# liruiw/GA-DDPG

Hardware: AMD Instinct MI355X
Metric: DDPG grad-steps/sec (B=256, N=1024 pts) (higher is better)
Workload: dtype f32 (3xbf16-split products, f32 accumulate)

## Files before the change

ga-ddpg_amd/csrc/gemm.hip:

```cpp
#include "common.hpp"
#include <mutex>
#include <type_traits>
#include <string.h>

typedef float f32x16 __attribute__((ext_vector_type(16)));

#ifndef GAD_STREAM_STORE_AUX
#define GAD_STREAM_STORE_AUX 0
#endif

#define KT 32

__device__ __forceinline__ float4 f4zero() { return make_float4(0.f, 0.f, 0.f, 0.f); }
__device__ __forceinline__ float4 f4sel(bool c, float4 a, float4 b) {
    return make_float4(c ? a.x : b.x, c ? a.y : b.y, c ? a.z : b.z, c ? a.w : b.w);
}
__device__ __forceinline__ float4 ldg4(const float* p) { return *reinterpret_cast<const float4*>(p); }

typedef unsigned gad_u32x4 __attribute__((ext_vector_type(4)));
__device__ __forceinline__ float4 buf_ld4(__amdgpu_buffer_rsrc_t r, int vo, int so) {
    const gad_u32x4 u = __builtin_amdgcn_raw_buffer_load_b128(r, vo, so, 0);
    return make_float4(__uint_as_float(u.x), __uint_as_float(u.y), __uint_as_float(u.z), __uint_as_float(u.w));
}
__device__ __forceinline__ float buf_ld(__amdgpu_buffer_rsrc_t r, int vo, int so) {
// ... 511 lines not shown
    float4 rb[UB];
    auto load_tile = [&](int kt) {
        const int k0 = kt * KT;
        const bool tail = k0 + KT > bulk;
#pragma unroll
        for (int it = 0; it < UA; ++it) {
            int i, kk; unit_T<BM>(it * 256 + tid, i, kk);
            const int r = row0 + i;
            const bool ok = r < n_rows && (k0 + kk < Kp);
            ra[it] = x_raw<XM>(x, r, ok, zoff, k0 + kk, tail, XM == 1 ? ptS[i] : 0);
        }
#pragma unroll
        for (int it = 0; it < UB; ++it) {
            int j, kk; unit_T<BN>(it * 256 + tid, j, kk);
            const int n = n0 + j;
            const bool ok = n < n_out && (k0 + kk < Kp);
            rb[it] = ldg4(Wg + (size_t)(ok ? n : 0) * Kp + (ok ? k0 + kk : 0));
        }
    };
    auto store_tile = [&](int kt) {
        const int k0 = kt * KT;
#pragma unroll
        for (int it = 0; it < UA; ++it) {
            int i, kk; unit_T<BM>(it * 256 + tid, i, kk);
            const int r = row0 + i;
            const bool ok = r < n_rows && (k0 + kk < Kp);
            store_T<BM>(As, i, kk, x_finish<XM>(x, ra[it], ok, k0 + kk, sv, tv));
        }
#pragma unroll
        for (int it = 0; it < UB; ++it) {
            int j, kk; unit_T<BN>(it * 256 + tid, j, kk);
            const bool ok = (n0 + j) < n_out && (k0 + kk < Kp);
            store_T<BN>(Bs, j, kk, f4sel(ok, rb[it], f4zero()));
        }
    };
    bool preloaded = false;
    if (XM == 0) { load_tile(0); preloaded = true; }
    if (XM == 0 && x.affine) stage_affine<256>(sv, tv, x, zoff, x.c_in);
    for (; row0 < n_rows; row0 += gridDim.x * BM) {
        f32x16 acc[TM][TN];
#pragma unroll
        for (int a = 0; a < TM; ++a)
#pragma unroll
            for (int b = 0; b < TN; ++b)
#pragma unroll
                for (int v = 0; v < 16; ++v) acc[a][b][v] = 0.f;
        if (tid < BM) {
            const int r = row0 + tid;
            wS[tid] = r < n_rows ? (row_w ? row_w[r] : 1.f) : 0.f;
            if (XM == 1) ptS[tid] = r < n_rows ? x.row_pt[r] : 0;
        }
        int pgl = -1, pg_before = -1, pg_after = -1;
        float psgn = 1.f;
        if (POOL) {
            const int r = row0 + lane;
            pgl = r < n_rows ? pe.row_grp[r] : -1;
            pg_before = row0 > 0 ? pe.row_grp[row0 - 1] : -1;
            pg_after = row0 + BM < n_rows ? pe.row_grp[row0 + BM] : -1;
            psgn = pe.gamma[n0 + lane] < 0.f ? -1.f : 1.f;
        }
        __syncthreads();
        if (!preloaded) load_tile(0);
        preloaded = false;
        for (int kt = 0; kt < nk; ++kt) {
            store_tile(kt);
            __syncthreads();
            if (kt + 1 < nk) load_tile(kt + 1);
            mfma_ktile<TM, TN, PA, PB>(As, Bs, wm * TM * 32, wn * TN * 32, lane, acc);
            __syncthreads();
        }
        const int l31 = lane & 31, half = lane >> 5;
        if (POOL) {
            static_assert(!POOL || (BM == 64 && BN == 64 && TM == 1 && TN == 1 && TILE >= 64 * 65), "pooled epilogue: 64 x 64 tiles");
            float* zt = smem;
#pragma unroll
            for (int v = 0; v < 16; ++v) zt[(wm * 32 + acc_row(v, half)) * 65 + wn * 32 + l31] = acc[0][0][v];
            __syncthreads();
            {
                const float sg1[1] = {psgn};
                pool_tile64<1>(zt + lane, 65, 0, pgl, row0, min(64, n_rows - row0), sg1, __builtin_amdgcn_readfirstlane(wave), 4,
                               __builtin_amdgcn_readfirstlane(pg_before), __builtin_amdgcn_readfirstlane(pg_after),
                               pe.key + n0 + lane, pe.C);
            }
        }
#pragma unroll
        for (int tn = 0; tn < TN; ++tn) {
            const int n = n0 + wn * TN * 32 + tn * 32 + l31;
            float s1 = 0.f, s2 = 0.f;
#pragma unroll
            for (int tm = 0; tm < TM; ++tm)
#pragma unroll
                for (int v = 0; v < 16; ++v) {
                    const int il = wm * TM * 32 + tm * 32 + acc_row(v, half);
                    const int r = row0 + il;
                    const float zv = acc[tm][tn][v];
                    if (zout && r < n_rows && n < n_out) zout[(size_t)r * zout_pitch + ooff + n] = zv;
                    const float w = wS[il];
                    s1 = fmaf(w, zv, s1);
                    s2 = fmaf(w * zv, zv, s2);
                }
            csum[tn] += s1;
            csq[tn] += s2;
        }
        __syncthreads();
    }
    if (stat_sum) {
        const int rep = DET ? blockIdx.x : blockIdx.x % GAD_STAT_REPLICAS;
        block_column_atomics<WM, WN, TN, DET>(smem, csum, csq, lane, wm, wn, n0, n_out,
                                              stat_sum + (size_t)rep * stat_stride + ooff,
                                              stat_sq + (size_t)rep * stat_stride + ooff);
    }
}

typedef float f32x2 __attribute__((ext_vector_type(2)));

typedef __bf16 gad_bf16x8 __attribute__((ext_vector_type(8)));
__device__ __forceinline__ unsigned gad_cvt_pk_bf16(float lo, float hi) {
    unsigned r;
    __asm__("v_cvt_pk_bf16_f32 %0, %1, %2" : "=v"(r) : "v"(lo), "v"(hi));
    return r;
}
__device__ __forceinline__ void gad_split2(float a, float b, unsigned& H, unsigned& M, unsigned& L) {
    H = gad_cvt_pk_bf16(a, b);
    const f32x2 r = f32x2{a, b} - f32x2{__uint_as_float(H << 16), __uint_as_float(H & 0xffff0000u)};
    M = gad_cvt_pk_bf16(r.x, r.y);
    const f32x2 q = r - f32x2{__uint_as_float(M << 16), __uint_as_float(M & 0xffff0000u)};
    L = gad_cvt_pk_bf16(q.x, q.y);
}
__device__ __forceinline__ gad_bf16x8 gad_as_bf16x8(gad_u32x4 u) { return *reinterpret_cast<gad_bf16x8*>(&u); }

static int g_opt_mfma_split = 0;
static int g_opt_deterministic = 0;
static bool split_on(int family) {
    return !g_opt_deterministic && (g_opt_mfma_split == GAD_SPLIT_ALL || (g_opt_mfma_split & family) != 0);
}

namespace spw {
constexpr int APL = 64 * 64, BPL = 128 * 64, STAGE = 3 * (APL + BPL);
struct BRegs { gad_u32x4 r[2][3]; };
__device__ __forceinline__ void load_b(BRegs& b, __amdgpu_buffer_rsrc_t rs, const int (&vb)[2], int plane_bytes, int kt) {
#pragma unroll
    for (int u = 0; u < 2; ++u)
#pragma unroll
        for (int p = 0; p < 3; ++p) b.r[u][p] = __builtin_amdgcn_raw_buffer_load_b128(rs, vb[u], p * plane_bytes + kt * 64, 0);
}
__device__ __forceinline__ void store_b(unsigned char* stage, const BRegs& b, int tid) {
    const int row = tid >> 2;
    unsigned char* q = stage + 3 * APL + row * 64 + ((((tid & 3) ^ ((row >> 2) & 3))) << 4);
#pragma unroll
    for (int u = 0; u < 2; ++u)
#pragma unroll
        for (int p = 0; p < 3; ++p) *reinterpret_cast<gad_u32x4*>(q + p * BPL + u * (64 * 64)) = b.r[u][p];
}
__device__ __forceinline__ void store_a4(unsigned char* stage, int row, int tid, float4 v, unsigned sg) {
    unsigned h0, m0, l0, h1, m1, l1;
    gad_split2(__uint_as_float(__float_as_uint(v.x) ^ sg), __uint_as_float(__float_as_uint(v.y) ^ sg), h0, m0, l0);
    gad_split2(__uint_as_float(__float_as_uint(v.z) ^ sg), __uint_as_float(__float_as_uint(v.w) ^ sg), h1, m1, l1);
    unsigned char* q = stage + row * 64 + (((((tid & 7) >> 1) ^ ((row >> 2) & 3))) << 4) + ((tid & 1) << 3);
    *reinterpret_cast<uint2*>(q) = make_uint2(h0, h1);
    *reinterpret_cast<uint2*>(q + APL) = make_uint2(m0, m1);
    *reinterpret_cast<uint2*>(q + 2 * APL) = make_uint2(l0, l1);
}
__device__ __forceinline__ void ktile(const unsigned char* stage, int arow, int brow, int fo, f32x16 (&acc)[2], f32x16 (&an)[2]) {
#pragma unroll
    for (int s = 0; s < 2; ++s) {
        const int off = fo ^ (s << 5);
        const unsigned char* ap = stage + arow + off;
        const unsigned char* bp = stage + 3 * APL + brow + off;
        const gad_u32x4 AH = *reinterpret_cast<const gad_u32x4*>(ap), AM = *reinterpret_cast<const gad_u32x4*>(ap + APL);
        const gad_u32x4 AL = *reinterpret_cast<const gad_u32x4*>(ap + 2 * APL);
        gad_u32x4 BH[2], BM[2], BL[2];
#pragma unroll
        for (int t = 0; t < 2; ++t) {
            BH[t] = *reinterpret_cast<const gad_u32x4*>(bp + t * (32 * 64));
            BM[t] = *reinterpret_cast<const gad_u32x4*>(bp + BPL + t * (32 * 64));
            BL[t] = *reinterpret_cast<const gad_u32x4*>(bp + 2 * BPL + t * (32 * 64));
        }
#define GAD_SPW(A, B)                                                                                                          \
        _Pragma("unroll") for (int t = 0; t < 2; ++t) {                                                                        \
            if (s) an[t] = __builtin_amdgcn_mfma_f32_32x32x16_bf16(gad_as_bf16x8(A), gad_as_bf16x8(B[t]), an[t], 0, 0, 0);     \
            else acc[t] = __builtin_amdgcn_mfma_f32_32x32x16_bf16(gad_as_bf16x8(A), gad_as_bf16x8(B[t]), acc[t], 0, 0, 0);     \
        }
        GAD_SPW(AL, BH) GAD_SPW(AH, BL) GAD_SPW(AM, BM) GAD_SPW(AM, BH) GAD_SPW(AH, BM) GAD_SPW(AH, BH)
#undef GAD_SPW
    }
}
}

template <int XM, bool POOL, bool SP = false>
__global__ __launch_bounds__(256, 2) void gemm_fwd_wide_kernel(XSrc x, const int32_t* __restrict__ n_rows_dev, int n_rows_static,
                                                               const float* __restrict__ row_w, const float* __restrict__ W,
                                                               int Kp, int n_out, float* __restrict__ zout, int zout_pitch,
                                                               double* __restrict__ stat_sum, double* __restrict__ stat_sq,
                                                               int stat_stride, PoolEpi pe, const uint16_t* __restrict__ wsp,
                                                               int wsp_pitch, int wsp_plane, unsigned long long* __restrict__ ts) {
    KTimer kt_(ts);
    GAD_WPH_DECL;
    GAD_WKL_DECL;
    constexpr int BM = 64, BN = 128, P = KT + 4, STAGE = SP ? spw::STAGE / 4 : (BM + BN) * P, VM = 512;
    static_assert(2 * STAGE >= 64 * 129, "the pooled epilogue's tile lives in the operand buffers");
    __shared__ __attribute__((aligned(16))) float smem[2 * STAGE + 2 * VM + BM + 4 * BM];
    float* sv = smem + 2 * STAGE;
    float* tv = sv + VM;
    float* wS = tv + VM;
    float* dxS = wS + BM;
    const int tid = threadIdx.x, lane = tid & 63;
    const int wave = __builtin_amdgcn_readfirstlane(tid >> 6);
    const int wm = wave >> 1, wn = wave & 1;
    const int l31 = lane & 31, half = lane >> 5;
    const int n0 = blockIdx.y * BN;
    const int n_rows = n_rows_dev ? min(*n_rows_dev, n_rows_static) : n_rows_static;
    if ((int)(blockIdx.x * BM) >= n_rows) return;
    const int nk = (XM == 0 ? Kp : x.feat_c) / KT;
    const int c4 = (tid & 7) * 4;
    const int ur = tid >> 3;
    const __amdgpu_buffer_rsrc_t ar_ = __builtin_amdgcn_make_buffer_rsrc(const_cast<float*>(XM == 0 ? x.zin : x.feat), 0, GAD_BUF_MAX, 0x00020000);
    const __amdgpu_buffer_rsrc_t wr_ = __builtin_amdgcn_make_buffer_rsrc(const_cast<float*>(W), 0, GAD_BUF_MAX, 0x00020000);
    const int zo_pitch4 = zout_pitch * 4;
    const __amdgpu_buffer_rsrc_t zo_ = __builtin_amdgcn_make_buffer_rsrc(zout ? zout : const_cast<float*>(W), 0, zout ? gad_nbytes(n_rows, zo_pitch4) : 0, 0x00020000);
    int vb[4];
#pragma unroll
    for (int u = 0; u < 4; ++u) vb[u] = ((n0 + ur + 32 * u) * Kp + c4) * 4;
    const __amdgpu_buffer_rsrc_t ws_ = __builtin_amdgcn_make_buffer_rsrc(const_cast<uint16_t*>(SP ? wsp : reinterpret_cast<const uint16_t*>(W)), 0, GAD_BUF_MAX, 0x00020000);
    int vbs[2];
#pragma unroll
    for (int u = 0; u < 2; ++u) vbs[u] = ((n0 + (tid >> 2) + 64 * u) * wsp_pitch + (tid & 3) * 8) * 2;
    unsigned char* const smem_b = reinterpret_cast<unsigned char*>(smem);
    const int sp_fo = ((half ^ ((l31 >> 2) & 3)) << 4);
    if (XM == 0) {
        if (x.bn.stat_sum) {
            const bool writer = blockIdx.x == 0 && blockIdx.y == 0;
            for (int i = tid; i < Kp; i += 256) {
                float sc, sh;
                gad_bn_fin_channel(x.bn, i, writer, sc, sh);
                sv[i] = sc; tv[i] = sh;
            }
        } else {
            stage_affine<256>(sv, tv, x, 0, Kp);
        }
    }

    float csum[2] = {0.f, 0.f}, csq[2] = {0.f, 0.f};
    for (int row0 = blockIdx.x * BM; row0 < n_rows; row0 += gridDim.x * BM) {
        f32x16 acc[2];
        f32x16 an[2];
#pragma unroll
        for (int t = 0; t < 2; ++t)
#pragma unroll
            for (int v = 0; v < 16; ++v) { acc[t][v] = 0.f; if (SP) an[t][v] = 0.f; }
        int pgl = -1, pg_before = -1, pg_after = -1;
        float psgn[2] = {1.f, 1.f};
        if (POOL) {
            const int r = row0 + lane;
            pgl = r < n_rows ? pe.row_grp[r] : -1;
            pg_before = row0 > 0 ? pe.row_grp[row0 - 1] : -1;
            pg_after = row0 + BM < n_rows ? pe.row_grp[row0 + BM] : -1;
            psgn[0] = pe.gamma[n0 + lane] < 0.f ? -1.f : 1.f;
            psgn[1] = pe.gamma[n0 + 64 + lane] < 0.f ? -1.f : 1.f;
        }
        const int ra0 = min(row0 + ur, max(n_rows - 1, 0)), ra1 = min(row0 + ur + 32, max(n_rows - 1, 0));
        const int va0 = ((XM == 0 ? ra0 * x.zin_pitch : x.row_pt[ra0] * x.feat_c) + c4) * 4;
        const int va1 = ((XM == 0 ? ra1 * x.zin_pitch : x.row_pt[ra1] * x.feat_c) + c4) * 4;
        float4 ra2[2][2], rb2[2][SP ? 1 : 4];
        spw::BRegs rbs[SP ? 2 : 1];
        auto load_regs = [&](int kt, auto setc) {
            constexpr int S = decltype(setc)::value;
            const int k0 = kt * (KT * 4);
            ra2[S][0] = buf_ld4(ar_, va0, k0); ra2[S][1] = buf_ld4(ar_, va1, k0);
            if (SP) { spw::load_b(rbs[SP ? S : 0], ws_, vbs, wsp_plane * 2, kt); return; }
#pragma unroll
            for (int u = 0; u < (SP ? 1 : 4); ++u) rb2[S][u] = buf_ld4(wr_, vb[u], k0);
        };
        auto write_lds = [&](int kt, auto setc) {
            constexpr int S = decltype(setc)::value;
            const float4* ra = ra2[S];
            const float4* rb = rb2[S];
            float* As = smem + (kt & 1) * STAGE;
            float* Bs = As + BM * P;
            float4 s4 = make_float4(1.f, 1.f, 1.f, 1.f), t4 = f4zero();
            if (XM == 0) {
                s4 = *reinterpret_cast<const float4*>(sv + kt * KT + c4);
                t4 = *reinterpret_cast<const float4*>(tv + kt * KT + c4);
            }
#pragma unroll
            for (int u = 0; u < 2; ++u) {
                float4 v = ra[u];
                if (XM == 0) {
                    v.x = fmaxf(fmaf(v.x, s4.x, t4.x), 0.f); v.y = fmaxf(fmaf(v.y, s4.y, t4.y), 0.f);
                    v.z = fmaxf(fmaf(v.z, s4.z, t4.z), 0.f); v.w = fmaxf(fmaf(v.w, s4.w, t4.w), 0.f);
                }
                if (SP) spw::store_a4(smem_b + (kt & 1) * spw::STAGE, ur + 32 * u, tid, v, (ur & 1) ? 0x80000000u : 0u);
                else *reinterpret_cast<float4*>(As + (ur + 32 * u) * P + c4) = v;
            }
            if (SP) { spw::store_b(smem_b + (kt & 1) * spw::STAGE, rbs[SP ? S : 0], tid); return; }
#pragma unroll
            for (int u = 0; u < (SP ? 1 : 4); ++u) *reinterpret_cast<float4*>(Bs + (ur + 32 * u) * P + c4) = rb[u];
        };
        const std::integral_constant<int, 0> S0;
        const std::integral_constant<int, 1> S1;
        load_regs(0, S0);
        if (nk > 1) load_regs(1, S1);
        __syncthreads();
        if (tid < BM) {
            const int r = row0 + tid;
            wS[tid] = r < n_rows ? (row_w ? row_w[r] : 1.f) : 0.f;
            if (XM == 1) {
                const int rr = min(r, max(n_rows - 1, 0));
                const float* p = x.src_xyz + (size_t)x.row_pt[rr] * 3;
                float q0 = p[0], q1 = p[1], q2 = p[2];
                if (x.ctr_xyz) {
                    const float* cp = x.ctr_xyz + (size_t)x.row_grp[rr] * 3;
                    q0 = __fsub_rn(q0, cp[0]); q1 = __fsub_rn(q1, cp[1]); q2 = __fsub_rn(q2, cp[2]);
                }
                *reinterpret_cast<float4*>(dxS + 4 * tid) = make_float4(q0, q1, q2, 0.f);
            }
        }
        GAD_WPH(1);
        write_lds(0, S0);
        if (nk > 2) load_regs(2, S0);
        __syncthreads();
        GAD_WPH(2);
        auto ktile = [&](int kt, auto nxtc) {
            if (SP) {
                GAD_WKL(0);
                spw::ktile(smem_b + (kt & 1) * spw::STAGE, (wm * 32 + l31) * 64, (wn * 64 + l31) * 64, sp_fo, acc, an);
                GAD_WKL(1);
                if (kt + 1 < nk) write_lds(kt + 1, nxtc);
                if (kt + 3 < nk) load_regs(kt + 3, nxtc);
                GAD_WKL(2);
                __syncthreads();
                GAD_WKL(3);
                return;
            }
            const float* As = smem + (kt & 1) * STAGE + (wm * 32 + l31) * P + 4 * half;
            const float* Bs = smem + (kt & 1) * STAGE + BM * P + (wn * 64 + l31) * P + 4 * half;
            float4 a4 = *reinterpret_cast<const float4*>(As);
            float4 b0 = *reinterpret_cast<const float4*>(Bs), b1 = *reinterpret_cast<const float4*>(Bs + 32 * P);
#pragma unroll
            for (int j = 0; j < KT / 8; ++j) {
                float4 an = a4, bn0 = b0, bn1 = b1;
                if (j + 1 < KT / 8) {
                    an = *reinterpret_cast<const float4*>(As + 8 * (j + 1));
                    bn0 = *reinterpret_cast<const float4*>(Bs + 8 * (j + 1));
                    bn1 = *reinterpret_cast<const float4*>(Bs + 32 * P + 8 * (j + 1));
                }
                acc[0] = __builtin_amdgcn_mfma_f32_32x32x2f32(a4.x, b0.x, acc[0], 0, 0, 0);
                acc[1] = __builtin_amdgcn_mfma_f32_32x32x2f32(a4.x, b1.x, acc[1], 0, 0, 0);
                acc[0] = __builtin_amdgcn_mfma_f32_32x32x2f32(a4.y, b0.y, acc[0], 0, 0, 0);
                acc[1] = __builtin_amdgcn_mfma_f32_32x32x2f32(a4.y, b1.y, acc[1], 0, 0, 0);
                acc[0] = __builtin_amdgcn_mfma_f32_32x32x2f32(a4.z, b0.z, acc[0], 0, 0, 0);
                acc[1] = __builtin_amdgcn_mfma_f32_32x32x2f32(a4.z, b1.z, acc[1], 0, 0, 0);
                acc[0] = __builtin_amdgcn_mfma_f32_32x32x2f32(a4.w, b0.w, acc[0], 0, 0, 0);
                acc[1] = __builtin_amdgcn_mfma_f32_32x32x2f32(a4.w, b1.w, acc[1], 0, 0, 0);
                a4 = an; b0 = bn0; b1 = bn1;
            }
            if (kt + 1 < nk) write_lds(kt + 1, nxtc);
            if (kt + 3 < nk) load_regs(kt + 3, nxtc);
            __syncthreads();
        };
        for (int kt = 0; kt < nk; kt += 2) {
            ktile(kt, S1);
            if (kt + 1 < nk) ktile(kt + 1, S0);
        }
        GAD_WPH(3);
        if (SP) {
#pragma unroll
            for (int t = 0; t < 2; ++t)
#pragma unroll
                for (int v = 0; v < 16; ++v) acc[t][v] = (v & 1) ? an[t][v] - acc[t][v] : acc[t][v] - an[t][v];
        }
        if (XM == 1) {
#pragma unroll
            for (int t = 0; t < 2; ++t) {
                const float* wx = W + (size_t)(n0 + wn * 64 + t * 32 + l31) * Kp + x.feat_c;
                const float w0 = wx[0], w1 = wx[1], w2 = wx[2];
#pragma unroll
                for (int v = 0; v < 16; ++v) {
                    const float4 q = *reinterpret_cast<const float4*>(dxS + 4 * (wm * 32 + acc_row(v, half)));
                    acc[t][v] = fmaf(q.x, w0, fmaf(q.y, w1, fmaf(q.z, w2, acc[t][v])));
                }
            }
        }
        if (POOL) {
            float* zt = smem;
#pragma unroll
            for (int t = 0; t < 2; ++t)
#pragma unroll
                for (int v = 0; v < 16; ++v) zt[(wm * 32 + acc_row(v, half)) * 129 + wn * 64 + t * 32 + l31] = acc[t][v];
            __syncthreads();
            const int gb = __builtin_amdgcn_readfirstlane(pg_before), ga = __builtin_amdgcn_readfirstlane(pg_after);
            pool_tile64<2>(zt + lane, 129, 64, pgl, row0, min(64, n_rows - row0), psgn, wave, 4, gb, ga, pe.key + n0 + lane, pe.C);
        }
        if (SP) {
#pragma unroll
        for (int t = 0; t < 2; ++t) {
            const int n = n0 + wn * 64 + t * 32 + l31;
            const int vzo = (4 * half * zout_pitch + n) * 4;
#pragma unroll
            for (int v = 0; v < 16; ++v)
                __builtin_amdgcn_raw_buffer_store_b32(__float_as_uint(acc[t][v]), zo_, vzo, (row0 + wm * 32 + (v & 3) + 8 * (v >> 2)) * zo_pitch4, 0);
        }
        __builtin_amdgcn_sched_barrier(0);
#pragma unroll
        for (int t = 0; t < 2; ++t) {
            float s1 = 0.f, s2 = 0.f;
#pragma unroll
            for (int v = 0; v < 16; ++v) {
                const float w = wS[wm * 32 + acc_row(v, half)];
                const float zv = acc[t][v];
                s1 = fmaf(w, zv, s1);
                s2 = fmaf(w * zv, zv, s2);
            }
            csum[t] += s1;
            csq[t] += s2;
        }
        } else {
#pragma unroll
        for (int t = 0; t < 2; ++t) {
            const int n = n0 + wn * 64 + t * 32 + l31;
            const int vzo = (4 * half * zout_pitch + n) * 4;
            float s1 = 0.f, s2 = 0.f;
#pragma unroll
            for (int v = 0; v < 16; ++v) {
                const int il = wm * 32 + acc_row(v, half);
                const float zv = acc[t][v];
                __builtin_amdgcn_raw_buffer_store_b32(__float_as_uint(zv), zo_, vzo, (row0 + wm * 32 + (v & 3) + 8 * (v >> 2)) * zo_pitch4, 0);
                const float w = wS[il];
                s1 = fmaf(w, zv, s1);
                s2 = fmaf(w * zv, zv, s2);
            }
            csum[t] += s1;
            csq[t] += s2;
        }
        }
        GAD_WPH(4);
    }
    if (stat_sum) {
        const int rep = blockIdx.x % GAD_STAT_REPLICAS;
        block_column_atomics<2, 2, 2>(smem, csum, csq, lane, wm, wn, n0, n_out, stat_sum + (size_t)rep * stat_stride,
                                      stat_sq + (size_t)rep * stat_stride);
    }
#ifdef GAD_W_PHASES
    __asm__ volatile("s_waitcnt vmcnt(0)" ::: "memory");
    GAD_WPH(5);
    GAD_WPH_STORE(ts);
    GAD_WKL_STORE(ts);
#endif
}

static int g_opt_fwd_wide = 1;
static int g_opt_dx_wide = 1, g_opt_dw_wide = 1;
static int g_opt_bwd_fused = 1;
static int g_opt_fwd_bn_prologue = 1;
static int g_opt_bwd_wide = 0;
static int g_opt_bwd_wide_slab = 4;
static int g_opt_dw_wide_wgs = 256;
static bool fits_i32_bytes(long long rows, int pitch_a, int pitch_b, int pitch_c, int pitch_d);
static bool fwd_wideable(const gad_gemm_fwd_args& a) {
    if (g_opt_deterministic || !g_opt_fwd_wide || a.n_groups != 1 || a.zin_off[0] != 0 || a.w_off[0] != 0 || a.out_off[0] != 0) return false;
    if (!fits_i32_bytes(a.n_rows, a.mode == 1 ? a.feat_c : a.zin_pitch, a.zout ? a.zout_pitch : 0, 0, 0)) return false;
    if (a.n_rows < 2048 || a.n_out[0] % 128 != 0 || a.ones_col >= 0) return false;
    if (a.mode == 2) return false;
    if (a.mode == 1)
        return g_opt_fwd_wide != 2 && !a.pool_key && a.act_c == 0 && a.feat_c % 32 == 0 && a.feat_c >= 32 && a.feat_c <= 512 &&
               a.Kp == ((a.feat_c + 3 + 7) & ~7);
    if (a.Kp % 32 != 0 || a.Kp > 512 || a.Kp != a.c_in) return false;
    return !a.extra && a.scale && a.shift && a.relu;
}
static bool fits_i32_bytes(long long rows, int pitch_a, int pitch_b, int pitch_c, int pitch_d) {
    int p = pitch_a > pitch_b ? pitch_a : pitch_b;
    p = p > pitch_c ? p : pitch_c;
    p = p > pitch_d ? p : pitch_d;
    return rows * (long long)p * 4 <= (1ll << 31);
}

template <int KJ, int TN, int XM, bool POOL, bool SP = false>
__global__ __launch_bounds__(512, 2) void gemm_fwd_stream_kernel(XSrc x, const int32_t* __restrict__ n_rows_dev,
                                                                  int n_rows_static, const float* __restrict__ row_w,
// ... 16 lines not shown
    constexpr int PB = 2 * KP + 16;
    __shared__ __attribute__((aligned(16))) float Ws[SP ? 3 * NO * PB / 4 : NO * PW];
    __shared__ __attribute__((aligned(16))) float sv[KP], tv[KP];
    __shared__ float red[2 * 8 * NO];
    __shared__ float pz[POOL ? 8 * 32 * 64 : 1];
    static_assert(!POOL || TN == 4, "pooled epilogue: 128 output columns");
    const int tid = threadIdx.x, lane = tid & 63;
    const int wave = __builtin_amdgcn_readfirstlane(tid >> 6);
    const int l31 = lane & 31, half = lane >> 5;
    const int n_rows = n_rows_dev ? min(*n_rows_dev, n_rows_static) : n_rows_static;
    const int n_slabs = (n_rows + 31) >> 5;
#if GAD_X_PHASES == 2
    long long st1, st2, st3, st4;
    __asm__ volatile("s_waitcnt lgkmcnt(0)" ::: "memory");
    GAD_PH_STAMP(st1);
#endif
    int stride = gridDim.x * 8;
    int slab = wave * gridDim.x + blockIdx.x;
    int slab_end = n_slabs;
    if (POOL) {
        const int nw = gridDim.x * 8, base = n_slabs / nw, rem = n_slabs - base * nw;
        slab_end = slab * base + min(slab, rem) + base + (slab < rem ? 1 : 0);
        slab = slab * base + min(slab, rem);
        stride = 1;
    }
    const bool store_z = zout != nullptr;
    const __amdgpu_buffer_rsrc_t zrsrc =
        __builtin_amdgcn_make_buffer_rsrc(store_z ? zout : const_cast<float*>(W), 0, store_z ? gad_nbytes(n_rows, NO * 4) : 0, 0x00020000);
    const int zlane = (4 * half * NO + l31) * 4;
    float psgn[2];
    PoolRun prun[2];
    const int range0 = slab * 32;
    int g_after = -1;
    if (POOL && slab < slab_end) {
        const int g0 = pe.row_grp[range0];
        const int part0 = range0 > 0 && pe.row_grp[range0 - 1] == g0;
        if (slab_end * 32 < n_rows) g_after = pe.row_grp[slab_end * 32];
#pragma unroll
        for (int p = 0; p < 2; ++p) {
            psgn[p] = pe.gamma[p * 64 + lane] < 0.f ? -1.f : 1.f;
            prun[p].g = g0; prun[p].part = part0; prun[p].v = -INFINITY; prun[p].row = range0;
        }
    }

    f32x2 csum[TN], csq[TN];
#pragma unroll
    for (int t = 0; t < TN; ++t) { csum[t] = f32x2{0.f, 0.f}; csq[t] = f32x2{0.f, 0.f}; }

    XRaw ra[NG], rn[NG];
    float4 w1f[RE ? 2 : 1][RE ? PK : 1];
    if (RE) {
#pragma unroll
        for (int b = 0; b < 2; ++b)
#pragma unroll
            for (int j = 0; j < PK; ++j) w1f[b][j] = ldg4(x.pre_W + (size_t)(32 * b + l31) * x.pre_Kp + 8 * j + 4 * half);
    }
    int pt_nxt = 0;
    auto load_pt = [&](int sl) {
        const int r = min(sl * 32 + l31, max(n_rows - 1, 0));
        return (GATHER && sl < n_slabs) ? x.row_pt[r] : 0;
    };
    auto load_slab = [&](int sl, int pt, XRaw (&dst)[NG]) {
        const int r = min(sl < n_slabs ? sl * 32 + l31 : 0, max(n_rows - 1, 0));
        if (GATHER) {
            struct F3 { float x, y, z; } __attribute__((packed, aligned(4)));
            const float4 f = ldg4(x.feat + (size_t)pt * 4);
            const F3 p = *reinterpret_cast<const F3*>(x.src_xyz + (size_t)pt * 3);
            const int grp = x.row_grp[r];
            float q0 = p.x, q1 = p.y, q2 = p.z;
            if (x.ctr_xyz) {
                const F3 c = *reinterpret_cast<const F3*>(x.ctr_xyz + (size_t)grp * 3);
                q0 = __fsub_rn(q0, c.x); q1 = __fsub_rn(q1, c.y); q2 = __fsub_rn(q2, c.z);
            }
            float a0 = 0.f, a1 = 0.f, a2 = 0.f, a3 = 0.f, a4 = 0.f, a5 = 0.f;
            if (x.action) {
                const float* ap = x.action + (size_t)(grp / x.gps) * 6;
                const F3 u = *reinterpret_cast<const F3*>(ap), v = *reinterpret_cast<const F3*>(ap + 3);
                a0 = u.x; a1 = u.y; a2 = u.z; a3 = v.x; a4 = v.y; a5 = v.z;
            }
#pragma unroll
            for (int j = 0; j < NG; ++j) {
                dst[j].a = f;
                if (j == 0) dst[j].s = make_float4(q0, q1, q2, a0);
                else dst[j].s = half ? make_float4(a5, 0.f, 0.f, 0.f) : make_float4(a1, a2, a3, a4);
            }
            return;
        }
#pragma unroll
        for (int j = 0; j < NG; ++j)
            dst[j] = x_raw<GATHER ? 1 : 0>(x, r, true, 0, SP ? 16 * (j >> 1) + 8 * half + 4 * (j & 1) : 8 * j + 4 * half, GATHER, pt);
    };
    auto lds_b = [&](int j, float4 (&b4)[TN]) {
#pragma unroll
        for (int t = 0; t < TN; ++t) b4[t] = *reinterpret_cast<const float4*>(Ws + (t * 32 + l31) * PW + 8 * j + 4 * half);
    };
    {
        const int pt0 = load_pt(slab);
        load_slab(slab, pt0, ra);
        pt_nxt = load_pt(slab + stride);
    }
    {
        constexpr int UNITS = NO * KJ * 2, UW = (UNITS + 511) / 512;
        float4 wr[UW];
#pragma unroll
        for (int it = 0; it < UW; ++it) {
            const int u = it * 512 + tid;
            wr[it] = ldg4(W + (size_t)(u < UNITS ? u : 0) * 4);
        }
#if GAD_X_PHASES == 2
        GAD_PH_STAMP(st2);
        __asm__ volatile("s_waitcnt vmcnt(0)" ::: "memory");
        GAD_PH_STAMP(st3);
#endif
        if (ACT && tid < KP) {
            float sc, sh;
            if (x.bn.stat_sum) gad_bn_fin_channel(x.bn, tid, blockIdx.x == 0, sc, sh);
            else { sc = x.scale[tid]; sh = x.shift[tid]; }
            sv[tid] = sc; tv[tid] = sh;
        }
#pragma unroll
        for (int it = 0; it < UW; ++it) {
            const int u = it * 512 + tid;
            const int n = u / (KJ * 2), c = (u % (KJ * 2)) * 4;
            if (SP) {
                unsigned h0, m0, l0, h1, m1, l1;
                gad_split2(wr[it].x, wr[it].y, h0, m0, l0);
                gad_split2(wr[it].z, wr[it].w, h1, m1, l1);
                unsigned char* wp = reinterpret_cast<unsigned char*>(Ws) + n * PB + c * 2;
                if (u < UNITS) {
                    *reinterpret_cast<uint2*>(wp) = make_uint2(h0, h1);
                    *reinterpret_cast<uint2*>(wp + NO * PB) = make_uint2(m0, m1);
                    *reinterpret_cast<uint2*>(wp + 2 * NO * PB) = make_uint2(l0, l1);
                }
            } else if (u < UNITS) *reinterpret_cast<float4*>(Ws + n * PW + c) = wr[it];
        }
    }
    __syncthreads();
#if GAD_X_PHASES == 2
    GAD_PH_STAMP(st4);
    if (ts && lane == 0) {
        auto c16 = [&](long long t) { const long long d = (t - kt_start) >> 2; return (unsigned long long)(d > 65535 ? 65535 : d); };
        ts[2 * (blockIdx.x * 8 + wave)] = c16(st1) | (c16(st2) << 16) | (c16(st3) << 32) | (c16(st4) << 48);
    }
#endif

#ifdef GAD_X_PHASES
    long long tA = 0, tB = 0, tC = 0, ph_top = 0, ph_mfma = 0, ph_epi = 0;
    int ph_n = 0;
    long long tP, tS;
    GAD_PH_STAMP(tP);
    tS = (long long)kt_start;
#endif
    for (; slab < slab_end; slab += stride) {
        load_slab(slab + stride, pt_nxt, rn);
        pt_nxt = load_pt(slab + 2 * stride);
        float4 w4[4];
#pragma unroll
        for (int q = 0; q < 4; ++q) {
            const int r0 = slab * 32 + 8 * q + 4 * half;
            w4[q] = row_w ? ldg4(row_w + (r0 + 3 < n_rows_static ? r0 : 0)) : make_float4(1.f, 1.f, 1.f, 1.f);
        }
        if (slab * 32 + 32 > n_rows) {
#pragma unroll
            for (int q = 0; q < 4; ++q) {
                float* wq = &w4[q].x;
#pragma unroll
                for (int e = 0; e < 4; ++e) wq[e] = (slab * 32 + 8 * q + 4 * half + e < n_rows) ? wq[e] : 0.f;
            }
        }
        int gl = -1;
        if (POOL) { const int rr = slab * 32 + l31; gl = rr < n_rows ? pe.row_grp[rr] : -1; }
        __asm__ volatile("" ::: "memory");
        f32x16 acc[TN];
#pragma unroll
        for (int t = 0; t < TN; ++t)
#pragma unroll
            for (int v = 0; v < 16; ++v) acc[t][v] = 0.f;
        float4 bn[TN];
        if (!SP) lds_b(0, bn);
        GAD_PH_STAMP(tA);
        if (SP) {
            const unsigned char* wp = reinterpret_cast<const unsigned char*>(Ws) + l31 * PB + 16 * half;
            constexpr int NS = SP ? KJ / 2 : 1;
            gad_u32x4 AH[NS], AM[NS], AL[NS];
#pragma unroll
            for (int sg = 0; sg < NS; ++sg) {
                unsigned ah[4], am[4], al[4];
#pragma unroll
                for (int e = 0; e < 2; ++e) {
                    const int c = 16 * sg + 8 * half + 4 * e;
                    const float4 s4 = *reinterpret_cast<const float4*>(sv + c), t4 = *reinterpret_cast<const float4*>(tv + c);
                    const float4 zr = ra[SP ? 2 * sg + e : 0].a;
                    const float a0 = __builtin_fmaxf(fmaf(zr.x, s4.x, t4.x), 0.f), a1 = __builtin_fmaxf(fmaf(zr.y, s4.y, t4.y), 0.f);
                    const float a2 = __builtin_fmaxf(fmaf(zr.z, s4.z, t4.z), 0.f), a3 = __builtin_fmaxf(fmaf(zr.w, s4.w, t4.w), 0.f);
                    gad_split2(a0, a1, ah[2 * e], am[2 * e], al[2 * e]);
                    gad_split2(a2, a3, ah[2 * e + 1], am[2 * e + 1], al[2 * e + 1]);
                }
                const unsigned sgn = ((sg ^ l31) & 1) ? 0x80008000u : 0u;
                AH[sg] = gad_u32x4{ah[0] ^ sgn, ah[1] ^ sgn, ah[2] ^ sgn, ah[3] ^ sgn};
                AM[sg] = gad_u32x4{am[0] ^ sgn, am[1] ^ sgn, am[2] ^ sgn, am[3] ^ sgn};
                AL[sg] = gad_u32x4{al[0] ^ sgn, al[1] ^ sgn, al[2] ^ sgn, al[3] ^ sgn};
            }
#pragma unroll
            for (int pp = 0; pp < TN / 2; ++pp) {
                f32x16 an[2];
#pragma unroll
                for (int i = 0; i < 2; ++i)
#pragma unroll
                    for (int v = 0; v < 16; ++v) an[i][v] = 0.f;
#pragma unroll
                for (int sg = 0; sg < NS; ++sg) {
                    gad_u32x4 BH[2], BM[2], BL[2];
#pragma unroll
                    for (int i = 0; i < 2; ++i) {
                        const unsigned char* q = wp + (2 * pp + i) * 32 * PB + 32 * sg;
                        BH[i] = *reinterpret_cast<const gad_u32x4*>(q);
                        BM[i] = *reinterpret_cast<const gad_u32x4*>(q + NO * PB);
                        BL[i] = *reinterpret_cast<const gad_u32x4*>(q + 2 * NO * PB);
                    }
#define GAD_SPLIT_MFMA(A, B)                                                                                                   \
                    _Pragma("unroll") for (int i = 0; i < 2; ++i) {                                                             \
                        if (sg & 1) an[i] = __builtin_amdgcn_mfma_f32_32x32x16_bf16(gad_as_bf16x8(A[sg]), gad_as_bf16x8(B[i]), an[i], 0, 0, 0); \
                        else acc[2 * pp + i] = __builtin_amdgcn_mfma_f32_32x32x16_bf16(gad_as_bf16x8(A[sg]), gad_as_bf16x8(B[i]), acc[2 * pp + i], 0, 0, 0); \
                    }
                    GAD_SPLIT_MFMA(AL, BH) GAD_SPLIT_MFMA(AH, BL) GAD_SPLIT_MFMA(AM, BM)
                    GAD_SPLIT_MFMA(AM, BH) GAD_SPLIT_MFMA(AH, BM) GAD_SPLIT_MFMA(AH, BH)
#undef GAD_SPLIT_MFMA
                }
#pragma unroll
                for (int i = 0; i < 2; ++i)
#pragma unroll
                    for (int v = 0; v < 16; ++v) acc[2 * pp + i][v] = (v & 1) ? an[i][v] - acc[2 * pp + i][v] : acc[2 * pp + i][v] - an[i][v];
            }
        }
        f32x16 zacc[RE ? 2 : 1];
        if (RE) {
#pragma unroll
            for (int b = 0; b < 2; ++b)
#pragma unroll
                for (int v = 0; v < 16; ++v) zacc[b][v] = 0.f;
#pragma unroll
            for (int j = 0; j < PK; ++j) {
                const float4 xb = x_finish<1>(x, ra[j], true, 8 * j + 4 * half, sv, tv);
#pragma unroll
                for (int b = 0; b < 2; ++b) zacc[b] = __builtin_amdgcn_mfma_f32_32x32x2f32(w1f[b][j].x, xb.x, zacc[b], 0, 0, 0);
#pragma unroll
                for (int b = 0; b < 2; ++b) zacc[b] = __builtin_amdgcn_mfma_f32_32x32x2f32(w1f[b][j].y, xb.y, zacc[b], 0, 0, 0);
#pragma unroll
                for (int b = 0; b < 2; ++b) zacc[b] = __builtin_amdgcn_mfma_f32_32x32x2f32(w1f[b][j].z, xb.z, zacc[b], 0, 0, 0);
#pragma unroll
                for (int b = 0; b < 2; ++b) zacc[b] = __builtin_amdgcn_mfma_f32_32x32x2f32(w1f[b][j].w, xb.w, zacc[b], 0, 0, 0);
            }
        }
#pragma unroll
        for (int j = 0; j < (SP ? 0 : KJ); ++j) {
            float4 b4[TN];
#pragma unroll
            for (int t = 0; t < TN; ++t) b4[t] = bn[t];
            float4 a4;
            if (ACT) {
                const float4 s4 = *reinterpret_cast<const float4*>(sv + 8 * j + 4 * half);
                const float4 t4 = *reinterpret_cast<const float4*>(tv + 8 * j + 4 * half);
                float4 zr;
                if (RE) zr = make_float4(zacc[j >> 2][4 * (j & 3)], zacc[j >> 2][4 * (j & 3) + 1], zacc[j >> 2][4 * (j & 3) + 2],
                                         zacc[j >> 2][4 * (j & 3) + 3]);
                else zr = ra[RE ? 0 : j].a;
                const f32x2 lo = f32x2{zr.x, zr.y} * f32x2{s4.x, s4.y} + f32x2{t4.x, t4.y};
                const f32x2 hi = f32x2{zr.z, zr.w} * f32x2{s4.z, s4.w} + f32x2{t4.z, t4.w};
                a4 = make_float4(__builtin_fmaxf(lo.x, 0.f), __builtin_fmaxf(lo.y, 0.f), __builtin_fmaxf(hi.x, 0.f),
                                 __builtin_fmaxf(hi.y, 0.f));
            } else {
                a4 = x_finish<1>(x, ra[RE ? 0 : j], true, 8 * j + 4 * half, sv, tv);
            }
            if (j + 1 < KJ) lds_b(j + 1, bn);
#pragma unroll
            for (int t = 0; t < TN; ++t) acc[t] = __builtin_amdgcn_mfma_f32_32x32x2f32(a4.x, b4[t].x, acc[t], 0, 0, 0);
#pragma unroll
            for (int t = 0; t < TN; ++t) acc[t] = __builtin_amdgcn_mfma_f32_32x32x2f32(a4.y, b4[t].y, acc[t], 0, 0, 0);
#pragma unroll
            for (int t = 0; t < TN; ++t) acc[t] = __builtin_amdgcn_mfma_f32_32x32x2f32(a4.z, b4[t].z, acc[t], 0, 0, 0);
#pragma unroll
            for (int t = 0; t < TN; ++t) acc[t] = __builtin_amdgcn_mfma_f32_32x32x2f32(a4.w, b4[t].w, acc[t], 0, 0, 0);
        }
        GAD_PH_STAMP(tB);
        const int zrow = slab * 32 * NO * 4;
        if (POOL) {
            float* zt = pz + wave * (32 * 64);
#pragma unroll
            for (int p = 0; p < 2; ++p) {
#pragma unroll
                for (int v = 0; v < 16; ++v) {
                    zt[acc_row(v, half) * 64 + l31] = acc[2 * p][v];
                    zt[acc_row(v, half) * 64 + 32 + l31] = acc[2 * p + 1][v];
                }
                pool_scan32(zt + lane, 64, gl, slab * 32, psgn[p], prun[p], pe.key + p * 64 + lane, pe.C);
            }
        }
#pragma unroll
        for (int v = 0; v < 16; v += 2) {
            const int rb = ((v & 3) + 8 * (v >> 2)) * NO * 4;
            const f32x2 wr = f32x2{(&w4[v >> 2].x)[v & 3], (&w4[v >> 2].x)[(v & 3) + 1]};
#pragma unroll
            for (int t = 0; t < TN; ++t) {
                const f32x2 zv = f32x2{acc[t][v], acc[t][v + 1]};
                if (store_z) {
                    __builtin_amdgcn_raw_buffer_store_b32(__float_as_uint(acc[t][v]), zrsrc, zlane + t * 128, zrow + rb, GAD_STREAM_STORE_AUX);
                    __builtin_amdgcn_raw_buffer_store_b32(__float_as_uint(acc[t][v + 1]), zrsrc, zlane + t * 128, zrow + rb + NO * 4, GAD_STREAM_STORE_AUX);
                }
                const f32x2 wz = wr * zv;
                csum[t] += wz;
                csq[t] += wz * zv;
            }
        }
#pragma unroll
        for (int j = 0; j < NG; ++j) ra[j] = rn[j];
#ifdef GAD_X_PHASES
        GAD_PH_STAMP(tC);
        ph_top += tA - tP; ph_mfma += tB - tA; ph_epi += tC - tB; tP = tC; ++ph_n;
#endif
    }
#ifdef GAD_X_PHASES
    if (ts && lane == 0) {
        const unsigned w = blockIdx.x * 8 + wave;
        if (GAD_X_PHASES != 2) ts[2 * w] = ((unsigned long long)ph_mfma << 32) | (unsigned long long)(ph_epi & 0xffffffffu);
        ts[2 * w + 1] = ((unsigned long long)ph_top << 32) | ((unsigned long long)(tP - tS) & 0xffffff00u) | (unsigned long long)ph_n;
    }
#endif
    if (POOL && range0 < slab_end * 32) {
#pragma unroll
        for (int p = 0; p < 2; ++p)
            if (prun[p].g >= 0)
                pool_put(pe.key + p * 64 + lane, prun[p].g, pe.C, prun[p].v, prun[p].row, prun[p].part != 0 || prun[p].g == g_after);
    }
    if (stat_sum) {
#pragma unroll
        for (int t = 0; t < TN; ++t) {
            const float c0 = csum[t].x + csum[t].y, c1 = csq[t].x + csq[t].y;
            const float s0 = c0 + __shfl_xor(c0, 32, 64);
            const float s1 = c1 + __shfl_xor(c1, 32, 64);
            if (lane < 32) { red[wave * NO + t * 32 + lane] = s0; red[(8 + wave) * NO + t * 32 + lane] = s1; }
        }
        __syncthreads();
        if (tid < NO) {
            float s0 = 0.f, s1 = 0.f;
#pragma unroll
            for (int w = 0; w < 8; ++w) { s0 += red[w * NO + tid]; s1 += red[(8 + w) * NO + tid]; }
            const int rep = blockIdx.x % GAD_STAT_REPLICAS;
            atomic_add_f64(stat_sum + (size_t)rep * stat_stride + tid, (double)s0);
            atomic_add_f64(stat_sq + (size_t)rep * stat_stride + tid, (double)s1);
        }
    }
}

#define SK_NW 8
#define SK_CH 6
#define SK_SP 36
#define SK_KCAP (8 * SK_NW * SK_CH * SK_MAXCH)
#define SK_MAXCH 3
template <int NW>
__global__ __launch_bounds__(64 * NW) void gemm_fwd_skinny_kernel(XSrc x, Groups gr, int n_rows,
                                                                     const float* __restrict__ row_w,
                                                                     const float* __restrict__ W, int Kp,
                                                                     float* __restrict__ zout, int zout_pitch,
                                                                     double* __restrict__ stat_sum,
                                                                     double* __restrict__ stat_sq, int stat_stride, unsigned long long* __restrict__ ts) {
    KTimer kt(ts);
    __shared__ __attribute__((aligned(16))) float stA[NW * 32 * SK_SP], stW[NW * 32 * SK_SP];
    __shared__ __attribute__((aligned(16))) float sv[SK_KCAP], tv[SK_KCAP];
    float* const part = stA;
    static_assert(32 * SK_SP >= 16 * 64, "partial tile must fit the wavefront's stage");
    const int tid = threadIdx.x, lane = tid & 63;
    const int wave = __builtin_amdgcn_readfirstlane(tid >> 6);
    const int l31 = lane & 31, half = lane >> 5;
    const int g = blockIdx.z;
    const int zoff = gr.aoff[g], n_out = gr.nout[g], ooff = gr.ooff[g];
    const int n0 = blockIdx.x * 32, row0 = blockIdx.y * 32;
    if (n0 >= n_out) return;
    const float* Wg = W + gr.woff[g] + (size_t)min(n0 + l31, n_out - 1) * Kp + 4 * half;
    const int r = min(row0 + l31, max(n_rows - 1, 0));
    const int nj = Kp >> 3;
    const int per = (nj + NW - 1) / NW;
    const int j0 = wave * per, j1 = min(nj, j0 + per);

    f32x16 acc;
#pragma unroll
    for (int v = 0; v < 16; ++v) acc[v] = 0.f;
    float* const myA = stA + wave * (32 * SK_SP);
    float* const myW = stW + wave * (32 * SK_SP);
    const int rsub = lane >> 3, chunk = lane & 7;
    const float* pa[4];
    const float* pw[4];
#pragma unroll
    for (int i = 0; i < 4; ++i) {
        pa[i] = x.zin + (size_t)min(row0 + rsub + 8 * i, max(n_rows - 1, 0)) * x.zin_pitch + zoff + 4 * chunk;
        pw[i] = W + gr.woff[g] + (size_t)min(n0 + rsub + 8 * i, n_out - 1) * Kp + 4 * chunk;
    }
    auto staged = [&](int jb) { return jb + 4 <= j1 && 8 * (jb + 4) <= x.c_in; };
    float4 ga[4], gw[4];
    auto load_blk = [&](int jb) {
#pragma unroll
        for (int i = 0; i < 4; ++i) { ga[i] = ldg4(pa[i] + 8 * jb); gw[i] = ldg4(pw[i] + 8 * jb); }
    };
    if (j0 < j1 && staged(j0)) load_blk(j0);
    if (x.bn.stat_sum) {
        const bool writer = blockIdx.x == 0 && blockIdx.y == 0;
        for (int i = tid; i < x.c_in; i += 64 * NW) {
            float sc, sh;
            gad_bn_fin_channel(x.bn, i, writer, sc, sh);
            sv[i] = sc;
            tv[i] = sh;
        }
    } else if (x.affine) stage_affine<64 * NW>(sv, tv, x, zoff, x.c_in);
    __syncthreads();
    for (int jb = j0; jb < j1; jb += 4) {
        if (staged(jb)) {
#pragma unroll
            for (int i = 0; i < 4; ++i) {
                *reinterpret_cast<float4*>(myA + (rsub + 8 * i) * SK_SP + 4 * chunk) = ga[i];
                *reinterpret_cast<float4*>(myW + (rsub + 8 * i) * SK_SP + 4 * chunk) = gw[i];
            }
            if (jb + 4 < j1 && staged(jb + 4)) load_blk(jb + 4);
            __builtin_amdgcn_fence(__ATOMIC_RELEASE, "wavefront");
            __builtin_amdgcn_wave_barrier();
            __builtin_amdgcn_fence(__ATOMIC_ACQUIRE, "wavefront");
#pragma unroll
            for (int u = 0; u < 4; ++u) {
                XRaw raw;
                raw.a = *reinterpret_cast<const float4*>(myA + l31 * SK_SP + 8 * u + 4 * half);
                raw.s = f4zero();
                const float4 a4 = x_finish<0>(x, raw, true, 8 * (jb + u) + 4 * half, sv, tv);
                const float4 b4 = *reinterpret_cast<const float4*>(myW + l31 * SK_SP + 8 * u + 4 * half);
                acc = __builtin_amdgcn_mfma_f32_32x32x2f32(a4.x, b4.x, acc, 0, 0, 0);
                acc = __builtin_amdgcn_mfma_f32_32x32x2f32(a4.y, b4.y, acc, 0, 0, 0);
                acc = __builtin_amdgcn_mfma_f32_32x32x2f32(a4.z, b4.z, acc, 0, 0, 0);
                acc = __builtin_amdgcn_mfma_f32_32x32x2f32(a4.w, b4.w, acc, 0, 0, 0);
            }
            __builtin_amdgcn_fence(__ATOMIC_RELEASE, "wavefront");
            __builtin_amdgcn_wave_barrier();
        } else {
            const int je = min(jb + 4, j1);
            XRaw ra[4];
            float4 rb[4];
#pragma unroll
            for (int u = 0; u < 4; ++u) {
                const int j = min(jb + u, nj - 1);
                const int col = 8 * j + 4 * half;
                ra[u] = x_raw<0>(x, r, true, zoff, col, col + 4 > x.c_in, 0);
                rb[u] = ldg4(Wg + 8 * j);
            }
            if (jb + 4 < j1 && staged(jb + 4)) load_blk(jb + 4);
#pragma unroll
            for (int u = 0; u < 4; ++u) {
                if (jb + u < je) {
                    const float4 a4 = x_finish<0>(x, ra[u], true, 8 * (jb + u) + 4 * half, sv, tv);
                    const float4 b4 = rb[u];
                    acc = __builtin_amdgcn_mfma_f32_32x32x2f32(a4.x, b4.x, acc, 0, 0, 0);
                    acc = __builtin_amdgcn_mfma_f32_32x32x2f32(a4.y, b4.y, acc, 0, 0, 0);
                    acc = __builtin_amdgcn_mfma_f32_32x32x2f32(a4.z, b4.z, acc, 0, 0, 0);
                    acc = __builtin_amdgcn_mfma_f32_32x32x2f32(a4.w, b4.w, acc, 0, 0, 0);
                }
            }
        }
    }
#pragma unroll
    for (int v = 0; v < 16; ++v) part[wave * (32 * SK_SP) + v * 64 + lane] = acc[v];
    __syncthreads();
    if (wave != 0) return;
#pragma unroll
// ... 735 lines not shown
        };
        lds_operands(0);
        for (; quad < n_quads; quad += gridDim.x) {
            slab = quad * 4 + wave;
            const int r_nn = row_of(slab + 8 * gridDim.x);
            const int grp_nn = GM == 1 ? d.row_grp[r_nn] : 0;
            const float w_nxt = d.row_w ? d.row_w[r_nxt] : 1.f;
            const bool row_live = slab * 32 + l31 < n_rows;
            f32x16 acc[2];
#pragma unroll
            for (int t = 0; t < 2; ++t)
#pragma unroll
                for (int v = 0; v < 16; ++v) acc[t][v] = 0.f;
            float zp[2][16];
            const int zrow = (slab < n_slabs ? slab : 0) * 32 * 64 * 4;
#pragma unroll
            for (int uu = 0; uu < NU; ++uu) {
                if (uu + AHEAD < NU) load_u(r_cur, grp_cur, uu + AHEAD, (uu + AHEAD) % RING);
                else load_u(r_nxt, grp_nxt, uu + AHEAD - NU, (uu + AHEAD) % RING);
                if (uu == 0) {
#pragma unroll
                    for (int v = 0; v < 16; ++v)
#pragma unroll
                        for (int t = 0; t < 2; ++t)
                            zp[t][v] = __uint_as_float(__builtin_amdgcn_raw_buffer_load_b32(
                                zrsrc, glane + t * 128, zrow + ((v & 3) + 8 * (v >> 2)) * 256, 0));
                }
                __builtin_amdgcn_sched_barrier(0);
                float* const hb = mybuf + (uu / (NU / 2)) * (4 * 32 * HP) + (uu % (NU / 2)) * 8;
                {
                    const float4 z = rz[uu % RING];
                    float4 g = rg[uu % RING];
                    if (GM == 1) {
                        const int4 a = ra[uu % RING];
                        const int rr = slab * 32 + l31;
                        g.x = a.x == rr ? g.x : 0.f; g.y = a.y == rr ? g.y : 0.f;
                        g.z = a.z == rr ? g.z : 0.f; g.w = a.w == rr ? g.w : 0.f;
                    }
                    float4 a4;
                    a4.x = P.x * g.x - wrow * fmaf(S.x, z.x, Q.x); a4.y = P.y * g.y - wrow * fmaf(S.y, z.y, Q.y);
                    a4.z = P.z * g.z - wrow * fmaf(S.z, z.z, Q.z); a4.w = P.w * g.w - wrow * fmaf(S.w, z.w, Q.w);
                    if (!row_live) a4 = make_float4(0.f, 0.f, 0.f, 0.f);
                    *reinterpret_cast<float4*>(hb) = a4;
                    const float4 b0 = nb0, b1 = nb1;
                    lds_operands((uu + 1) % NU);
                    acc[0] = __builtin_amdgcn_mfma_f32_32x32x2f32(a4.x, b0.x, acc[0], 0, 0, 0);
                    acc[1] = __builtin_amdgcn_mfma_f32_32x32x2f32(a4.x, b1.x, acc[1], 0, 0, 0);
                    acc[0] = __builtin_amdgcn_mfma_f32_32x32x2f32(a4.y, b0.y, acc[0], 0, 0, 0);
                    acc[1] = __builtin_amdgcn_mfma_f32_32x32x2f32(a4.y, b1.y, acc[1], 0, 0, 0);
                    acc[0] = __builtin_amdgcn_mfma_f32_32x32x2f32(a4.z, b0.z, acc[0], 0, 0, 0);
                    acc[1] = __builtin_amdgcn_mfma_f32_32x32x2f32(a4.z, b1.z, acc[1], 0, 0, 0);
                    acc[0] = __builtin_amdgcn_mfma_f32_32x32x2f32(a4.w, b0.w, acc[0], 0, 0, 0);
                    acc[1] = __builtin_amdgcn_mfma_f32_32x32x2f32(a4.w, b1.w, acc[1], 0, 0, 0);
                }
                if ((uu + 1) % (NU / 2) == 0) __syncthreads();
            }
            const bool full = slab * 32 + 32 <= n_rows;
#pragma unroll
            for (int v = 0; v < 16; ++v) {
                const int row = acc_row(v, half);
                const bool live = slab * 32 + row < n_rows;
                const int rb = zrow + ((v & 3) + 8 * (v >> 2)) * 256;
#pragma unroll
                for (int t = 0; t < 2; ++t) {
                    const float gv = acc[t][v];
                    const float zv = zp[t][v];
                    const bool act = fmaf(zv, ps[t], pt[t]) > 0.f && live;
                    const float ga = act ? gv : 0.f;
                    if (full) __builtin_amdgcn_raw_buffer_store_b32(__float_as_uint(ga), grsrc, glane + t * 128, rb, GAD_STREAM_STORE_AUX);
                    else if (live) e.gout[(size_t)(slab * 32 + row) * 64 + t * 32 + l31] = ga;
                    sb[t] += ga;
                    sg[t] = fmaf(ga, (zv - pm[t]) * pi[t], sg[t]);
                }
            }
            r_cur = r_nxt; r_nxt = r_nn;
            grp_cur = grp_nxt; grp_nxt = grp_nn;
            wrow = w_nxt;
        }
#pragma unroll
        for (int t = 0; t < 2; ++t) {
            const float s0 = sb[t] + __shfl_xor(sb[t], 32, 64);
            const float s1 = sg[t] + __shfl_xor(sg[t], 32, 64);
            if (lane < 32) { red[wave * 64 + t * 32 + lane] = s0; red[(4 + wave) * 64 + t * 32 + lane] = s1; }
        }
    } else {
        const int q = wave - 4;
        const int b = q & 1;
        const int tcl = NCT == 2 ? (q >> 1) : 0;
        const int s0 = NCT == 2 ? 0 : 2 * (q >> 1);
        constexpr int NS = NCT == 2 ? 4 : 2;
        const float psb = e.ps[32 * b + l31], ptb = e.pt[32 * b + l31];
        f32x16 aw[2];
#pragma unroll
        for (int h = 0; h < 2; ++h)
#pragma unroll
            for (int v = 0; v < 16; ++v) aw[h][v] = 0.f;
        float yq[NS][16];
        auto load_y = [&](int slab, int s) {
            const int zrow = (slab < n_slabs ? slab : 0) * 32 * 64 * 4;
#pragma unroll
            for (int v = 0; v < 16; ++v)
                yq[s][v] = __uint_as_float(__builtin_amdgcn_raw_buffer_load_b32(zrsrc, glane + b * 128, zrow + ((v & 3) + 8 * (v >> 2)) * 256, 0));
        };
        const float* const rbase = dzb + (4 * half) * HP + 32 * tcl + l31;
#pragma unroll
        for (int s = 0; s < NS; ++s) load_y(blockIdx.x * 4 + s0 + s, s);
        for (int quad = blockIdx.x; quad < n_quads; quad += gridDim.x) {
#pragma unroll
            for (int h = 0; h < 2; ++h) {
                __syncthreads();
#pragma unroll
                for (int s = 0; s < NS; ++s) {
                    const float* rb = rbase + (h * 4 + s0 + s) * (32 * HP);
                    float dz[16];
#pragma unroll
                    for (int v = 0; v < 16; ++v) dz[v] = rb[((v & 3) + 8 * (v >> 2)) * HP];
                    if (h == 0) {
#pragma unroll
                        for (int v = 0; v < 16; ++v) yq[s][v] = fmaxf(fmaf(yq[s][v], psb, ptb), 0.f);
                    }
#pragma unroll
                    for (int v = 0; v < 16; ++v) aw[h] = __builtin_amdgcn_mfma_f32_32x32x2f32(dz[v], yq[s][v], aw[h], 0, 0, 0);
                    if (h == 1) load_y((quad + gridDim.x) * 4 + s0 + s, s);
                }
            }
        }
        float* pout = partial + (size_t)(NCT == 2 ? blockIdx.x : 2 * blockIdx.x + (q >> 1)) * NO * 64;
#pragma unroll
        for (int h = 0; h < 2; ++h)
#pragma unroll
            for (int v = 0; v < 16; ++v) pout[(32 * (NCT * h + tcl) + acc_row(v, half)) * 64 + 32 * b + l31] = aw[h][v];
    }
    __syncthreads();
    if (tid < 64) {
        float s0 = 0.f, s1 = 0.f;
#pragma unroll
        for (int w = 0; w < 4; ++w) { s0 += red[w * 64 + tid]; s1 += red[(4 + w) * 64 + tid]; }
        const int rep = blockIdx.x % GAD_STAT_REPLICAS;
        atomic_add_f64(e.dbeta + (size_t)rep * e.stat_stride + tid, (double)s0);
        atomic_add_f64(e.dgamma + (size_t)rep * e.stat_stride + tid, (double)s1);
    }
}

template <int NJ, int GM, bool DW>
__global__ __launch_bounds__(512, 2) void gemm_bwd_stream_split_kernel(DzSrc d, const int32_t* __restrict__ n_rows_dev, int n_rows_static,
                                                                        const uint16_t* __restrict__ wsp, int wsp_plane, DxEpi e,
                                                                        float* __restrict__ partial, unsigned long long* __restrict__ ts) {
    KTimer kt(ts);
    constexpr int NO = 8 * NJ, NS = NO / 16;
    constexpr int HC = NO / 2, NCT = HC / 32;
    constexpr int RB = 2 * NO + 16, WPL = 64 * RB;
    constexpr int XSL = HC * 64, XPL = 4 * XSL, XBUF = 3 * XPL;
    __shared__ __attribute__((aligned(16))) unsigned char WtS[3 * WPL];
    __shared__ __attribute__((aligned(16))) float vec[3 * NO];
    __shared__ float red[2 * 8 * 64];
    __shared__ __attribute__((aligned(16))) unsigned char dzb[DW ? 2 * XBUF : 16];
    const int tid = threadIdx.x, lane = tid & 63;
    const int wave = __builtin_amdgcn_readfirstlane(tid >> 6);
    const int l31 = lane & 31, half = lane >> 5;
    const int n_rows = n_rows_dev ? min(*n_rows_dev, n_rows_static) : n_rows_static;
    {
        constexpr int CPR = NO / 8, UNITS = 3 * 64 * CPR, UW = (UNITS + 511) / 512;
        gad_u32x4 wr[UW];
#pragma unroll
        for (int it = 0; it < UW; ++it) {
            const int u = it * 512 + tid, uc = u < UNITS ? u : 0;
            const int pl = uc / (64 * CPR), rem = uc % (64 * CPR);
            wr[it] = *reinterpret_cast<const gad_u32x4*>(wsp + (size_t)pl * wsp_plane + (size_t)rem * 8);
        }
#pragma unroll
        for (int it = 0; it < UW; ++it) {
            const int u = it * 512 + tid;
            const int pl = u / (64 * CPR), rem = u % (64 * CPR), k = rem / CPR, c = rem % CPR;
            if (u < UNITS) *reinterpret_cast<gad_u32x4*>(WtS + pl * WPL + k * RB + c * 16) = wr[it];
        }
    }
    for (int i = tid; i < NO; i += 512) {
        float P, Q, S;
        dz_coef(d, i, P, Q, S, first_workgroup());
        vec[i] = P; vec[NO + i] = Q; vec[2 * NO + i] = S;
    }
    __syncthreads();
    const int n_slabs = (n_rows + 31) >> 5;
    const int n_quads = (n_slabs + 3) >> 2;
    const __amdgpu_buffer_rsrc_t zrsrc =
        __builtin_amdgcn_make_buffer_rsrc(const_cast<float*>(e.zprev), 0, gad_nbytes(n_rows, 64 * 4), 0x00020000);
    const int glane = (4 * half * 64 + l31) * 4;
    const int nprod = DW ? 4 : 8;

    if (!DW || wave < 4) {
        float ps[2], pt[2], pm[2], pi[2];
#pragma unroll
        for (int tk = 0; tk < 2; ++tk) {
            const int k = tk * 32 + l31;
            ps[tk] = e.ps[k]; pt[tk] = e.pt[k]; pm[tk] = e.pm[k]; pi[tk] = e.pi[k];
        }
        const __amdgpu_buffer_rsrc_t grsrc = __builtin_amdgcn_make_buffer_rsrc(e.gout, 0, gad_nbytes(n_rows, 64 * 4), 0x00020000);
        float sb[2] = {0.f, 0.f}, sg[2] = {0.f, 0.f};
        constexpr int NU = NO / 8, RING = 8, AHEAD = 6, RINGG = GM == 1 ? 4 : RING, AHEADG = GM == 1 ? 2 : AHEAD;
        static_assert(NU % RING == 0 && NU % RINGG == 0, "a slab's entries must fill the rings a whole number of times");
        float4 rz[RING], rg[RINGG];
        int4 ra[RINGG];
        auto row_of = [&](int sl) { return min(sl < n_slabs ? sl * 32 + l31 : 0, max(n_rows - 1, 0)); };
        auto load_z = [&](int r, int uu) {
            const unsigned n = 16 * (uu >> 1) + 8 * half + 4 * (uu & 1);
            rz[uu % RING] = ldg4(d.z + ((unsigned)r * NO + n));
            if (GM == 0) rg[uu % RINGG] = ldg4(d.G + ((unsigned)r * NO + n));
        };
        auto load_g = [&](int grp, int uu) {
            const unsigned n = 16 * (uu >> 1) + 8 * half + 4 * (uu & 1);
            ra[uu % RINGG] = *reinterpret_cast<const int4*>(d.argmax + ((unsigned)grp * NO + n));
            rg[uu % RINGG] = ldg4(d.dout + ((unsigned)grp * NO + n));
        };
        const int round_stride = DW ? 4 * gridDim.x : 8 * gridDim.x;
        int slab = DW ? blockIdx.x * 4 + wave : wave * gridDim.x + blockIdx.x;
        const int slab_limit = DW ? n_quads * 4 : n_slabs;
        int r_cur = row_of(slab), r_nxt = row_of(slab + round_stride);
        int grp_cur = GM == 1 ? d.row_grp[r_cur] : 0, grp_nxt = GM == 1 ? d.row_grp[r_nxt] : 0;
        float wrow = d.row_w ? d.row_w[r_cur] : 1.f;
#pragma unroll
        for (int i = 0; i < AHEAD; ++i) load_z(r_cur, i);
        if (GM == 1) {
#pragma unroll
            for (int i = 0; i < AHEADG; ++i) load_g(grp_cur, i);
        }
        const unsigned psel = (l31 & 1) ? 0x03020706u : 0x05040100u;
        const unsigned rsg = (l31 & 1) ? 0x80000000u : 0u;
        const int xq = l31 >> 3, xin = ((l31 >> 1) & 3) * 4;
        const unsigned char* const wb = WtS + l31 * RB + 16 * half;
        for (; slab < slab_limit; slab += round_stride) {
            const int r_nn = row_of(slab + 2 * round_stride);
            const int grp_nn = GM == 1 ? d.row_grp[r_nn] : 0;
            const float w_nxt = d.row_w ? d.row_w[r_nxt] : 1.f;
            const bool row_live = slab * 32 + l31 < n_rows;
            f32x16 acc[2], an[2];
#pragma unroll
            for (int t = 0; t < 2; ++t)
#pragma unroll
                for (int v = 0; v < 16; ++v) { acc[t][v] = 0.f; an[t][v] = 0.f; }
            float zp[2][16];
            const int zrow = (slab < n_slabs ? slab : 0) * 32 * 64 * 4;
#pragma unroll
            for (int s2 = 0; s2 < NS; ++s2) {
#pragma unroll
                for (int ee = 0; ee < 2; ++ee) {
                    const int uu = 2 * s2 + ee + AHEAD;
                    if (uu < NU) load_z(r_cur, uu); else load_z(r_nxt, uu - NU);
                    if (GM == 1) {
                        const int ug = 2 * s2 + ee + AHEADG;
                        if (ug < NU) load_g(grp_cur, ug); else load_g(grp_nxt, ug - NU);
                    }
                }
                if (s2 == 0) {
#pragma unroll
                    for (int v = 0; v < 16; ++v)
#pragma unroll
                        for (int t = 0; t < 2; ++t)
                            zp[t][v] = __uint_as_float(__builtin_amdgcn_raw_buffer_load_b32(
                                zrsrc, glane + t * 128, zrow + ((v & 3) + 8 * (v >> 2)) * 256, 0));
                }
                __builtin_amdgcn_sched_barrier(0);
                gad_u32x4 BH[2], BM[2], BL[2];
#pragma unroll
                for (int t = 0; t < 2; ++t) {
                    const unsigned char* q = wb + t * (32 * RB) + 32 * s2;
                    BH[t] = *reinterpret_cast<const gad_u32x4*>(q);
                    BM[t] = *reinterpret_cast<const gad_u32x4*>(q + WPL);
                    BL[t] = *reinterpret_cast<const gad_u32x4*>(q + 2 * WPL);
                }
                unsigned ah[4], am[4], al[4];
#pragma unroll
                for (int ee = 0; ee < 2; ++ee) {
                    const int uu = 2 * s2 + ee;
                    const int n = 16 * s2 + 8 * half + 4 * ee;
                    const float4 P = *reinterpret_cast<const float4*>(vec + n);
                    const float4 Q = *reinterpret_cast<const float4*>(vec + NO + n);
                    const float4 S = *reinterpret_cast<const float4*>(vec + 2 * NO + n);
                    const float4 z = rz[uu % RING];
                    float4 g = rg[uu % RINGG];
                    if (GM == 1) {
                        const int4 a = ra[uu % RINGG];
                        const int rr = slab * 32 + l31;
                        g.x = a.x == rr ? g.x : 0.f; g.y = a.y == rr ? g.y : 0.f;
                        g.z = a.z == rr ? g.z : 0.f; g.w = a.w == rr ? g.w : 0.f;
                    }
                    float4 a4;
                    a4.x = P.x * g.x - wrow * fmaf(S.x, z.x, Q.x); a4.y = P.y * g.y - wrow * fmaf(S.y, z.y, Q.y);
                    a4.z = P.z * g.z - wrow * fmaf(S.z, z.z, Q.z); a4.w = P.w * g.w - wrow * fmaf(S.w, z.w, Q.w);
                    if (!row_live) a4 = make_float4(0.f, 0.f, 0.f, 0.f);
                    gad_split2(__uint_as_float(__float_as_uint(a4.x) ^ rsg), __uint_as_float(__float_as_uint(a4.y) ^ rsg), ah[2 * ee], am[2 * ee], al[2 * ee]);
                    gad_split2(__uint_as_float(__float_as_uint(a4.z) ^ rsg), __uint_as_float(__float_as_uint(a4.w) ^ rsg), ah[2 * ee + 1], am[2 * ee + 1], al[2 * ee + 1]);
                }
                const gad_u32x4 AH = {ah[0], ah[1], ah[2], ah[3]}, AM = {am[0], am[1], am[2], am[3]}, AL = {al[0], al[1], al[2], al[3]};
                if (DW) {
                    unsigned char* hb = dzb + (s2 / (NS / 2)) * XBUF + wave * XSL + xin;
                    const int cbase = (16 * s2 + 8 * half) % HC + (l31 & 1);
#pragma unroll
                    for (int i = 0; i < 4; ++i) {
                        const int cl = cbase + 2 * i;
                        unsigned char* q = hb + cl * 64 + ((xq ^ ((cl >> 2) & 3)) << 4);
                        const unsigned own[3] = {ah[i], am[i], al[i]};
#pragma unroll
                        for (int pl = 0; pl < 3; ++pl) {
                            const unsigned nbr = (unsigned)__builtin_amdgcn_update_dpp(0, (int)own[pl], 0xB1, 0xf, 0xf, false);
                            *reinterpret_cast<unsigned*>(q + pl * XPL) = __builtin_amdgcn_perm(nbr, own[pl], psel);
                        }
                    }
                }
#define GAD_SPB(A, B)                                                                                                          \
                _Pragma("unroll") for (int t = 0; t < 2; ++t) {                                                                \
                    if (s2 & 1) an[t] = __builtin_amdgcn_mfma_f32_32x32x16_bf16(gad_as_bf16x8(A), gad_as_bf16x8(B[t]), an[t], 0, 0, 0);   \
                    else acc[t] = __builtin_amdgcn_mfma_f32_32x32x16_bf16(gad_as_bf16x8(A), gad_as_bf16x8(B[t]), acc[t], 0, 0, 0); \
                }
                GAD_SPB(AL, BH) GAD_SPB(AH, BL) GAD_SPB(AM, BM) GAD_SPB(AM, BH) GAD_SPB(AH, BM) GAD_SPB(AH, BH)
#undef GAD_SPB
                if (DW && (s2 + 1) % (NS / 2) == 0) __syncthreads();
            }
            const bool full = slab * 32 + 32 <= n_rows;
#pragma unroll
            for (int v = 0; v < 16; ++v) {
                const int row = acc_row(v, half);
                const bool live = slab * 32 + row < n_rows;
                const int rb = zrow + ((v & 3) + 8 * (v >> 2)) * 256;
#pragma unroll
                for (int t = 0; t < 2; ++t) {
                    const float gv = (v & 1) ? an[t][v] - acc[t][v] : acc[t][v] - an[t][v];
                    const float zv = live ? zp[t][v] : 0.f;
                    const bool act = fmaf(zv, ps[t], pt[t]) > 0.f && live;
                    const float ga = act ? gv : 0.f;
                    if (full) __builtin_amdgcn_raw_buffer_store_b32(__float_as_uint(ga), grsrc, glane + t * 128, rb, GAD_STREAM_STORE_AUX);
                    else if (live) e.gout[(size_t)(slab * 32 + row) * 64 + t * 32 + l31] = ga;
                    sb[t] += ga;
                    sg[t] = fmaf(ga, (zv - pm[t]) * pi[t], sg[t]);
                }
            }
            r_cur = r_nxt; r_nxt = r_nn;
            grp_cur = grp_nxt; grp_nxt = grp_nn;
            wrow = w_nxt;
        }
#pragma unroll
        for (int t = 0; t < 2; ++t) {
            const float s0 = sb[t] + __shfl_xor(sb[t], 32, 64);
            const float s1 = sg[t] + __shfl_xor(sg[t], 32, 64);
            if (lane < 32) { red[wave * 64 + t * 32 + lane] = s0; red[(8 + wave) * 64 + t * 32 + lane] = s1; }
        }
    } else {
        const int q = wave - 4;
        const int b = q & 1;
        const int tcl = NCT == 2 ? (q >> 1) : 0;
        const int s0 = NCT == 2 ? 0 : 2 * (q >> 1);
        constexpr int NSC = NCT == 2 ? 4 : 2;
        const float psb = e.ps[32 * b + l31], ptb = e.pt[32 * b + l31];
        f32x16 aw[2], awn[2];
#pragma unroll
        for (int h = 0; h < 2; ++h)
#pragma unroll
            for (int v = 0; v < 16; ++v) { aw[h][v] = 0.f; awn[h][v] = 0.f; }
        const int ylane = (8 * half * 64 + 32 * b + l31) * 4;
        float yr[NSC][16];
        gad_u32x4 YH[NSC][2], YM[NSC][2], YL[NSC][2];
        auto load_y = [&](int slab, int sl) {
            const int zrow = (slab < n_slabs ? slab : 0) * 32 * 64 * 4;
#pragma unroll
            for (int v = 0; v < 16; ++v)
                yr[sl][v] = __uint_as_float(__builtin_amdgcn_raw_buffer_load_b32(zrsrc, ylane, zrow + (16 * (v >> 3) + (v & 7)) * 256, 0));
        };
        const int cl = 32 * tcl + l31;
        const unsigned char* const rbase = dzb + cl * 64;
        const int fo = ((half ^ ((cl >> 2) & 3)) << 4);
#pragma unroll
        for (int sl = 0; sl < NSC; ++sl) load_y(blockIdx.x * 4 + s0 + sl, sl);
        for (int quad = blockIdx.x; quad < n_quads; quad += gridDim.x) {
#pragma unroll
            for (int h = 0; h < 2; ++h) {
                __syncthreads();
#pragma unroll
                for (int sl = 0; sl < NSC; ++sl) {
                    if (h == 0) {
#pragma unroll
                        for (int st = 0; st < 2; ++st) {
                            unsigned yh[4], ym[4], yl[4];
#pragma unroll
                            for (int i = 0; i < 4; ++i) {
                                float y0 = fmaxf(fmaf(yr[sl][8 * st + 2 * i], psb, ptb), 0.f), y1 = fmaxf(fmaf(yr[sl][8 * st + 2 * i + 1], psb, ptb), 0.f);
                                if (st) y0 = -y0; else y1 = -y1;
                                gad_split2(y0, y1, yh[i], ym[i], yl[i]);
                            }
                            YH[sl][st] = gad_u32x4{yh[0], yh[1], yh[2], yh[3]};
                            YM[sl][st] = gad_u32x4{ym[0], ym[1], ym[2], ym[3]};
                            YL[sl][st] = gad_u32x4{yl[0], yl[1], yl[2], yl[3]};
                        }
                    }
                    const unsigned char* rb = rbase + h * XBUF + (s0 + sl) * XSL;
#pragma unroll
                    for (int st = 0; st < 2; ++st) {
                        const int off = fo ^ (st << 5);
                        const gad_u32x4 AH = *reinterpret_cast<const gad_u32x4*>(rb + off);
                        const gad_u32x4 AM = *reinterpret_cast<const gad_u32x4*>(rb + XPL + off);
                        const gad_u32x4 AL = *reinterpret_cast<const gad_u32x4*>(rb + 2 * XPL + off);
#define GAD_SPC(A, B)                                                                                                          \
                        if (st) awn[h] = __builtin_amdgcn_mfma_f32_32x32x16_bf16(gad_as_bf16x8(A), gad_as_bf16x8(B[sl][st]), awn[h], 0, 0, 0); \
                        else aw[h] = __builtin_amdgcn_mfma_f32_32x32x16_bf16(gad_as_bf16x8(A), gad_as_bf16x8(B[sl][st]), aw[h], 0, 0, 0);
                        GAD_SPC(AL, YH) GAD_SPC(AH, YL) GAD_SPC(AM, YM) GAD_SPC(AM, YH) GAD_SPC(AH, YM) GAD_SPC(AH, YH)
#undef GAD_SPC
                    }
                    if (h == 1) load_y((quad + gridDim.x) * 4 + s0 + sl, sl);
                }
            }
        }
        float* pout = partial + (size_t)(NCT == 2 ? blockIdx.x : 2 * blockIdx.x + (q >> 1)) * NO * 64;
#pragma unroll
        for (int h = 0; h < 2; ++h)
#pragma unroll
            for (int v = 0; v < 16; ++v) pout[(32 * (NCT * h + tcl) + acc_row(v, half)) * 64 + 32 * b + l31] = aw[h][v] - awn[h][v];
    }
    __syncthreads();
    if (tid < 64) {
        float s0 = 0.f, s1 = 0.f;
        for (int w = 0; w < nprod; ++w) { s0 += red[w * 64 + tid]; s1 += red[(8 + w) * 64 + tid]; }
        const int rep = blockIdx.x % GAD_STAT_REPLICAS;
        atomic_add_f64(e.dbeta + (size_t)rep * e.stat_stride + tid, (double)s0);
        atomic_add_f64(e.dgamma + (size_t)rep * e.stat_stride + tid, (double)s1);
    }
}

template <int GM, int SC, bool SP = false>
__global__ __launch_bounds__(256, 2) void gemm_dx_wide_kernel(DzSrc d, const int32_t* __restrict__ n_rows_dev, int n_rows_static,
                                                              const float* __restrict__ W, int Kp, int n_out, DxEpi e,
                                                              const uint16_t* __restrict__ wsp, int wsp_plane,
                                                              unsigned long long* __restrict__ ts) {
    KTimer kt_(ts);
    constexpr int BM = 64, BN = 128, P = KT + 4, PB = BN + 4, STAGE = SP ? spw::STAGE / 4 : BM * P + KT * PB, VM = 512;
    __shared__ __attribute__((aligned(16))) float smem[2 * STAGE + 3 * VM + BM];
    __shared__ int32_t ptS[BM];
    float* vP = smem + 2 * STAGE;
    float* wS = vP + 3 * VM;
    int32_t* grS = reinterpret_cast<int32_t*>(wS);
    const int tid = threadIdx.x, lane = tid & 63;
    const int wave = __builtin_amdgcn_readfirstlane(tid >> 6);
    const int wm = wave >> 1, wn = wave & 1;
    const int l31 = lane & 31, half = lane >> 5;
    const int k0out = blockIdx.y * BN;
    const int n_rows = n_rows_dev ? min(*n_rows_dev, n_rows_static) : n_rows_static;
    if ((int)(blockIdx.x * BM) >= n_rows) return;
    const int nk = n_out / KT;
    const int gpitch = GM == 0 ? d.g_pitch : d.c;
    const __amdgpu_buffer_rsrc_t zr = __builtin_amdgcn_make_buffer_rsrc(const_cast<float*>(d.z), 0, GAD_BUF_MAX, 0x00020000);
    const __amdgpu_buffer_rsrc_t gr_ = __builtin_amdgcn_make_buffer_rsrc(const_cast<float*>(GM == 0 ? d.G : d.dout), 0, GAD_BUF_MAX, 0x00020000);
    const __amdgpu_buffer_rsrc_t ar = __builtin_amdgcn_make_buffer_rsrc(const_cast<int32_t*>(GM == 0 ? d.row_grp : d.argmax), 0, GAD_BUF_MAX, 0x00020000);
    const __amdgpu_buffer_rsrc_t wr = __builtin_amdgcn_make_buffer_rsrc(const_cast<float*>(W), 0, GAD_BUF_MAX, 0x00020000);
    const int zp_pitch4 = SC ? 0 : e.zprev_pitch * 4, go_pitch4 = SC ? 0 : e.gout_pitch * 4;
    const __amdgpu_buffer_rsrc_t pr = __builtin_amdgcn_make_buffer_rsrc(const_cast<float*>(SC ? W : e.zprev), 0, SC ? 0 : gad_nbytes(n_rows, zp_pitch4), 0x00020000);
    const __amdgpu_buffer_rsrc_t or_ = __builtin_amdgcn_make_buffer_rsrc(SC ? const_cast<float*>(W) : e.gout, 0, SC ? 0 : gad_nbytes(n_rows, go_pitch4), 0x00020000);
    const int c4 = (tid & 7) * 4, ur = tid >> 3;
    const int bk4 = (tid & 31) * 4, bn = tid >> 5;
    int vw[4];
#pragma unroll
    for (int u = 0; u < 4; ++u) vw[u] = ((bn + 8 * u) * Kp + k0out + bk4) * 4;
    const __amdgpu_buffer_rsrc_t ws_ = __builtin_amdgcn_make_buffer_rsrc(const_cast<uint16_t*>(SP ? wsp : reinterpret_cast<const uint16_t*>(W)), 0, GAD_BUF_MAX, 0x00020000);
    int vbs[2];
#pragma unroll
    for (int u = 0; u < 2; ++u) vbs[u] = ((k0out + (tid >> 2) + 64 * u) * n_out + (tid & 3) * 8) * 2;
    unsigned char* const smem_b = reinterpret_cast<unsigned char*>(smem);
    const int sp_fo = ((half ^ ((l31 >> 2) & 3)) << 4);
    for (int i = tid; i < n_out; i += 256) {
        float Pc, Qc, Sc;
        dz_coef(d, i, Pc, Qc, Sc, first_workgroup());
        vP[i] = Pc; vP[VM + i] = Qc; vP[2 * VM + i] = Sc;
    }
    (void)grS;
    float ps[2] = {0.f, 0.f}, pt[2] = {0.f, 0.f}, pm[2] = {0.f, 0.f}, pi[2] = {0.f, 0.f};
#pragma unroll
    for (int t = 0; t < 2; ++t) {
        const int k = k0out + wn * 64 + t * 32 + l31;
        if (!SC) { ps[t] = e.ps[k]; pt[t] = e.pt[k]; pm[t] = e.pm[k]; pi[t] = e.pi[k]; }
    }
    float cb[2] = {0.f, 0.f}, cg[2] = {0.f, 0.f};
    for (int row0 = blockIdx.x * BM; row0 < n_rows; row0 += gridDim.x * BM) {
        f32x16 acc[2];
        f32x16 an[2];
#pragma unroll
        for (int t = 0; t < 2; ++t)
#pragma unroll
            for (int v = 0; v < 16; ++v) { acc[t][v] = 0.f; if (SP) an[t][v] = 0.f; }
        int vz[2], vg[2];
        float wrow[2];
        bool live[2];
#pragma unroll
        for (int u = 0; u < 2; ++u) {
            const int r = row0 + ur + 32 * u;
            live[u] = r < n_rows;
            const int rr = live[u] ? r : max(n_rows - 1, 0);
            wrow[u] = d.row_w ? d.row_w[rr] : 1.f;
            vz[u] = (rr * d.z_pitch + c4) * 4;
            vg[u] = ((GM == 1 ? d.row_grp[rr] : rr) * gpitch + c4) * 4;
        }
        float4 rz[2], rg[2], rb[SP ? 1 : 4];
        gad_u32x4 ra[2];
        spw::BRegs rbs;
        auto load_regs = [&](int kt) {
#pragma unroll
            for (int u = 0; u < 2; ++u) {
                rz[u] = buf_ld4(zr, vz[u], kt * (KT * 4));
                rg[u] = buf_ld4(gr_, vg[u], kt * (KT * 4));
                if (GM == 1) ra[u] = __builtin_amdgcn_raw_buffer_load_b128(ar, vg[u], kt * (KT * 4), 0);
            }
            if (SP) { spw::load_b(rbs, ws_, vbs, wsp_plane * 2, kt); return; }
#pragma unroll
            for (int u = 0; u < (SP ? 1 : 4); ++u) rb[u] = buf_ld4(wr, vw[u], kt * (KT * 4) * Kp);
        };
        auto write_lds = [&](int kt) {
            float* As = smem + (kt & 1) * STAGE;
            float* Bs = As + BM * P;
            const int nb = kt * KT + c4;
            const float4 P4 = *reinterpret_cast<const float4*>(vP + nb), Q4 = *reinterpret_cast<const float4*>(vP + VM + nb);
            const float4 S4 = *reinterpret_cast<const float4*>(vP + 2 * VM + nb);
#pragma unroll
            for (int u = 0; u < 2; ++u) {
                float4 g = rg[u];
                const float4 z = rz[u];
                if (GM == 1) {
                    const unsigned r = row0 + ur + 32 * u;
                    g.x = ra[u].x == r ? g.x : 0.f; g.y = ra[u].y == r ? g.y : 0.f;
                    g.z = ra[u].z == r ? g.z : 0.f; g.w = ra[u].w == r ? g.w : 0.f;
                }
                const float w = wrow[u];
                float4 v;
                v.x = P4.x * g.x - w * fmaf(S4.x, z.x, Q4.x); v.y = P4.y * g.y - w * fmaf(S4.y, z.y, Q4.y);
                v.z = P4.z * g.z - w * fmaf(S4.z, z.z, Q4.z); v.w = P4.w * g.w - w * fmaf(S4.w, z.w, Q4.w);
                if (!live[u]) v = f4zero();
                if (SP) spw::store_a4(smem_b + (kt & 1) * spw::STAGE, ur + 32 * u, tid, v, (ur & 1) ? 0x80000000u : 0u);
                else *reinterpret_cast<float4*>(As + (ur + 32 * u) * P + c4) = v;
            }
            if (SP) { spw::store_b(smem_b + (kt & 1) * spw::STAGE, rbs, tid); return; }
#pragma unroll
            for (int u = 0; u < (SP ? 1 : 4); ++u)
                *reinterpret_cast<float4*>(Bs + (bn + 8 * u) * PB + bk4) = rb[u];
        };
        load_regs(0);
        __syncthreads();
        if (SC && tid < BM) ptS[tid] = e.row_pt[min(row0 + tid, max(n_rows - 1, 0))];
        write_lds(0);
        if (nk > 1) load_regs(1);
        __syncthreads();
        for (int kt = 0; kt < nk; ++kt) {
            if (SP) {
                spw::ktile(smem_b + (kt & 1) * spw::STAGE, (wm * 32 + l31) * 64, (wn * 64 + l31) * 64, sp_fo, acc, an);
                if (kt + 1 < nk) write_lds(kt + 1);
                if (kt + 2 < nk) load_regs(kt + 2);
                __syncthreads();
                continue;
            }
            const float* As = smem + (kt & 1) * STAGE + (wm * 32 + l31) * P + 4 * half;
            const float* Bs = smem + (kt & 1) * STAGE + BM * P + (4 * half) * PB + wn * 64 + l31;
            float4 a4 = *reinterpret_cast<const float4*>(As);
            float4 b0 = make_float4(Bs[0], Bs[PB], Bs[2 * PB], Bs[3 * PB]);
            float4 b1 = make_float4(Bs[32], Bs[PB + 32], Bs[2 * PB + 32], Bs[3 * PB + 32]);
#pragma unroll
            for (int j = 0; j < KT / 8; ++j) {
                float4 an = a4, bn0 = b0, bn1 = b1;
                if (j + 1 < KT / 8) {
                    an = *reinterpret_cast<const float4*>(As + 8 * (j + 1));
                    const float* bq = Bs + 8 * (j + 1) * PB;
                    bn0 = make_float4(bq[0], bq[PB], bq[2 * PB], bq[3 * PB]);
                    bn1 = make_float4(bq[32], bq[PB + 32], bq[2 * PB + 32], bq[3 * PB + 32]);
                }
                acc[0] = __builtin_amdgcn_mfma_f32_32x32x2f32(a4.x, b0.x, acc[0], 0, 0, 0);
                acc[1] = __builtin_amdgcn_mfma_f32_32x32x2f32(a4.x, b1.x, acc[1], 0, 0, 0);
                acc[0] = __builtin_amdgcn_mfma_f32_32x32x2f32(a4.y, b0.y, acc[0], 0, 0, 0);
                acc[1] = __builtin_amdgcn_mfma_f32_32x32x2f32(a4.y, b1.y, acc[1], 0, 0, 0);
                acc[0] = __builtin_amdgcn_mfma_f32_32x32x2f32(a4.z, b0.z, acc[0], 0, 0, 0);
                acc[1] = __builtin_amdgcn_mfma_f32_32x32x2f32(a4.z, b1.z, acc[1], 0, 0, 0);
                acc[0] = __builtin_amdgcn_mfma_f32_32x32x2f32(a4.w, b0.w, acc[0], 0, 0, 0);
                acc[1] = __builtin_amdgcn_mfma_f32_32x32x2f32(a4.w, b1.w, acc[1], 0, 0, 0);
                a4 = an; b0 = bn0; b1 = bn1;
            }
            if (kt + 1 < nk) write_lds(kt + 1);
            if (kt + 2 < nk) load_regs(kt + 2);
            __syncthreads();
        }
        if (SP) {
#pragma unroll
            for (int t = 0; t < 2; ++t)
#pragma unroll
                for (int v = 0; v < 16; ++v) acc[t][v] = (v & 1) ? an[t][v] - acc[t][v] : acc[t][v] - an[t][v];
        }
        if (SC) {
#pragma unroll
            for (int t = 0; t < 2; ++t) {
                const int k = k0out + wn * 64 + t * 32 + l31;
#pragma unroll
                for (int v = 0; v < 16; ++v) {
                    const int il = wm * 32 + acc_row(v, half);
                    if (row0 + il < n_rows) atomic_add_f32(e.dfeat + (size_t)ptS[il] * e.feat_c + k, acc[t][v]);
                }
            }
            continue;
        }
        const int rb0 = row0 + wm * 32;
#pragma unroll
        for (int t = 0; t < 2; ++t) {
            const int kcol = k0out + wn * 64 + t * 32 + l31;
            const int vzp = (4 * half * e.zprev_pitch + kcol) * 4, vgo = (4 * half * e.gout_pitch + kcol) * 4;
            float zp[16];
#pragma unroll
            for (int v = 0; v < 16; ++v) zp[v] = buf_ld(pr, vzp, (rb0 + (v & 3) + 8 * (v >> 2)) * zp_pitch4);
            const float npm = -pm[t] * pi[t];
            float sb = 0.f, sg = 0.f;
#pragma unroll
            for (int v = 0; v < 16; ++v) {
                const float ga = fmaf(zp[v], ps[t], pt[t]) > 0.f ? acc[t][v] : 0.f;
                __builtin_amdgcn_raw_buffer_store_b32(__float_as_uint(ga), or_, vgo, (rb0 + (v & 3) + 8 * (v >> 2)) * go_pitch4, 0);
                sb += ga;
                sg = fmaf(ga, fmaf(zp[v], pi[t], npm), sg);
            }
            cb[t] += sb; cg[t] += sg;
        }
    }
    if (SC) return;
    const int rep = blockIdx.x % GAD_STAT_REPLICAS;
    block_column_atomics<2, 2, 2>(smem, cb, cg, lane, wm, wn, k0out, e.k_valid, e.dbeta + (size_t)rep * e.stat_stride,
                                  e.dgamma + (size_t)rep * e.stat_stride);
}

__global__ __launch_bounds__(256) void dx_action_stream_kernel(DzSrc d, const int32_t* __restrict__ n_rows_dev, int n_rows_static,
                                                               const float* __restrict__ W, int Kp, int c0, DxEpi e,
                                                               unsigned long long* __restrict__ ts) {
    KTimer kt(ts);
    const int tid = threadIdx.x, lane = tid & 63;
    const int n_rows = n_rows_dev ? min(*n_rows_dev, n_rows_static) : n_rows_static;
    const int n_waves = gridDim.x * 4;
    const int gw = blockIdx.x * 4 + (tid >> 6);
    int chunk = (n_rows + n_waves - 1) / n_waves;
    chunk = (chunk + 3) & ~3;
    const int r0 = gw * chunk, r1 = min(n_rows, r0 + chunk);
    if (r0 >= r1) return;
    const int sub = lane >> 4, c4 = (lane & 15) * 4;
    float4 P, Q, S;
    dz_coef(d, c4 + 0, P.x, Q.x, S.x); dz_coef(d, c4 + 1, P.y, Q.y, S.y);
    dz_coef(d, c4 + 2, P.z, Q.z, S.z); dz_coef(d, c4 + 3, P.w, Q.w, S.w);
    float4 wa[6];
#pragma unroll
    for (int a = 0; a < 6; ++a)
        wa[a] = make_float4(W[(size_t)(c4 + 0) * Kp + c0 + a], W[(size_t)(c4 + 1) * Kp + c0 + a], W[(size_t)(c4 + 2) * Kp + c0 + a],
                            W[(size_t)(c4 + 3) * Kp + c0 + a]);
    double run[6] = {0.0, 0.0, 0.0, 0.0, 0.0, 0.0};
    int cur = -1;
    auto flush = [&]() {
        if (cur >= 0 && lane == 0)
#pragma unroll
            for (int a = 0; a < 6; ++a) atomic_add_f64(e.daction + (size_t)cur * 6 + a, run[a]);
#pragma unroll
        for (int a = 0; a < 6; ++a) run[a] = 0.0;
    };
    for (int rb = r0; rb < r1; rb += 4) {
        const int r = rb + sub;
        const bool live = r < r1;
        const int rr = live ? r : r1 - 1;
        const float4 z = ldg4(d.z + (size_t)rr * d.z_pitch + c4);
        const float4 g = ldg4(d.G + (size_t)rr * d.g_pitch + c4);
        const float w = d.row_w ? d.row_w[rr] : 1.f;
        const int smp = e.row_grp[rr] / e.gps;
        float4 dz;
        dz.x = P.x * g.x - w * fmaf(S.x, z.x, Q.x); dz.y = P.y * g.y - w * fmaf(S.y, z.y, Q.y);
        dz.z = P.z * g.z - w * fmaf(S.z, z.z, Q.z); dz.w = P.w * g.w - w * fmaf(S.w, z.w, Q.w);
        float p[6];
#pragma unroll
        for (int a = 0; a < 6; ++a) {
            p[a] = fmaf(dz.x, wa[a].x, fmaf(dz.y, wa[a].y, fmaf(dz.z, wa[a].z, dz.w * wa[a].w)));
            p[a] = live ? p[a] : 0.f;
#pragma unroll
            for (int m = 8; m >= 1; m >>= 1) p[a] += __shfl_xor(p[a], m, 16);
        }
        const int s0 = __builtin_amdgcn_readlane(smp, 0), s1 = __builtin_amdgcn_readlane(smp, 16);
        const int s2 = __builtin_amdgcn_readlane(smp, 32), s3 = __builtin_amdgcn_readlane(smp, 48);
        if (s0 == s1 && s1 == s2 && s2 == s3) {
            if (s0 != cur) { flush(); cur = s0; }
#pragma unroll
            for (int a = 0; a < 6; ++a) {
                float t = p[a] + __shfl_xor(p[a], 16, 64);
                t += __shfl_xor(t, 32, 64);
                run[a] += (double)t;
            }
        } else {
            flush();
            cur = -1;
            if ((lane & 15) == 0 && live)
#pragma unroll
                for (int a = 0; a < 6; ++a) atomic_add_f64(e.daction + (size_t)smp * 6 + a, (double)p[a]);
        }
    }
    flush();
}

static bool dx_action_streamable(const gad_gemm_dx_args& a, bool vec) {
    if (g_opt_deterministic || !g_opt_dx_stream || !vec || a.n_groups != 1 || a.dz_off[0] != 0 || a.w_off[0] != 0) return false;
    if (a.epilogue != 1 || a.dfeat || !a.daction || a.act_c != 6 || !a.row_grp || a.n_rows < 32768 || a.n_out[0] != 64) return false;
    const gad_dz_src& d = a.dz;
    return d.gmode == 0 && d.G && d.z && d.z_pitch % 4 == 0 && d.g_pitch % 4 == 0 && d.premasked && d.coefP && d.coefQ && d.coefS &&
           a.feat_c + 3 + a.act_c <= a.Kp;
// ... 967 lines not shown
    if (r_begin >= r_end) return;
    for (int i = tid; i < BT; i += 256) {
        float Pc, Qc, Sc;
        dz_coef(d, n0 + i, Pc, Qc, Sc, blockIdx.y == 0 && k0 == 0);
        vP[i] = Pc; vP[VM + i] = Qc; vP[2 * VM + i] = Sc;
        if (XM == 0) { sv[i] = x.scale[k0 + i]; tv[i] = x.shift[k0 + i]; }
    }
    const bool coords = XM == 1 && k0 == 0;
    float wx[4][3];
#pragma unroll
    for (int j = 0; j < 4; ++j) { wx[j][0] = 0.f; wx[j][1] = 0.f; wx[j][2] = 0.f; }
    f32x16 acc[2][2];
#pragma unroll
    for (int a = 0; a < 2; ++a)
#pragma unroll
        for (int b = 0; b < 2; ++b)
#pragma unroll
            for (int v = 0; v < 16; ++v) acc[a][b][v] = 0.f;
    const int c4 = (tid & 31) * 4, sr = tid >> 5;
    const int gpitch = GM == 0 ? d.g_pitch : d.c;
    float4 rz[4], rg[4], rx[4];
    int4 ra[4];
    float rw[4], rd[4][3];
    int pq[4], gq[4];
    int gd[4];
    auto load_idx = [&](int rb0) {
#pragma unroll
        for (int u = 0; u < 4; ++u) {
            const int r = rb0 + sr + 8 * u;
            const int rr = r < r_end ? r : r_end - 1;
            pq[u] = XM == 1 ? x.row_pt[rr] : 0;
            gq[u] = (XM == 1 && x.ctr_xyz) ? x.row_grp[rr] : 0;
            gd[u] = GM == 1 ? d.row_grp[rr] : 0;
        }
    };
    auto load_regs = [&](int rb0) {
#pragma unroll
        for (int u = 0; u < 4; ++u) {
            const int r = rb0 + sr + 8 * u;
            const int rr = r < r_end ? r : r_end - 1;
            rw[u] = d.row_w ? d.row_w[rr] : 1.f;
            rz[u] = ldg4(d.z + (size_t)rr * d.z_pitch + n0 + c4);
            if (GM == 0) {
                rg[u] = ldg4(d.G + (size_t)rr * gpitch + n0 + c4);
            } else {
                const int grp = gd[u];
                ra[u] = *reinterpret_cast<const int4*>(d.argmax + (size_t)grp * gpitch + n0 + c4);
                rg[u] = ldg4(d.dout + (size_t)grp * gpitch + n0 + c4);
            }
            if (XM == 0) {
                rx[u] = ldg4(x.zin + (size_t)rr * x.zin_pitch + k0 + c4);
            } else {
                rx[u] = ldg4(x.feat + (size_t)pq[u] * x.feat_c + k0 + c4);
                if (coords) {
                    const float* p = x.src_xyz + (size_t)pq[u] * 3;
                    float q0 = p[0], q1 = p[1], q2 = p[2];
                    if (x.ctr_xyz) {
                        const float* cp = x.ctr_xyz + (size_t)gq[u] * 3;
                        q0 = __fsub_rn(q0, cp[0]); q1 = __fsub_rn(q1, cp[1]); q2 = __fsub_rn(q2, cp[2]);
                    }
                    rd[u][0] = q0; rd[u][1] = q1; rd[u][2] = q2;
                }
            }
        }
        if (XM == 1 || GM == 1) load_idx(rb0 + KT);
    };
    auto write_lds = [&](int it, int rb0) {
        float* As = smem + (it & 1) * STAGE;
        float* Bs = As + KT * P;
        const float4 Pv = *reinterpret_cast<const float4*>(vP + c4), Qv = *reinterpret_cast<const float4*>(vP + VM + c4);
        const float4 Sv = *reinterpret_cast<const float4*>(vP + 2 * VM + c4);
        float4 s4 = f4zero(), t4 = f4zero();
        if (XM == 0) { s4 = *reinterpret_cast<const float4*>(sv + c4); t4 = *reinterpret_cast<const float4*>(tv + c4); }
#pragma unroll
        for (int u = 0; u < 4; ++u) {
            const int r = rb0 + sr + 8 * u;
            float4 g = rg[u];
            const float4 z = rz[u];
            if (GM == 1) {
                g.x = ra[u].x == r ? g.x : 0.f; g.y = ra[u].y == r ? g.y : 0.f;
                g.z = ra[u].z == r ? g.z : 0.f; g.w = ra[u].w == r ? g.w : 0.f;
            }
            const float w = rw[u];
            float4 a, b;
            a.x = Pv.x * g.x - w * fmaf(Sv.x, z.x, Qv.x); a.y = Pv.y * g.y - w * fmaf(Sv.y, z.y, Qv.y);
            a.z = Pv.z * g.z - w * fmaf(Sv.z, z.z, Qv.z); a.w = Pv.w * g.w - w * fmaf(Sv.w, z.w, Qv.w);
            if (XM == 0) {
                b.x = fmaxf(fmaf(rx[u].x, s4.x, t4.x), 0.f); b.y = fmaxf(fmaf(rx[u].y, s4.y, t4.y), 0.f);
                b.z = fmaxf(fmaf(rx[u].z, s4.z, t4.z), 0.f); b.w = fmaxf(fmaf(rx[u].w, s4.w, t4.w), 0.f);
            } else {
                b = rx[u];
            }
            if (r >= r_end) { a = f4zero(); b = f4zero(); }
            if (coords) {
#pragma unroll
                for (int dd = 0; dd < 3; ++dd) {
                    wx[0][dd] = fmaf(a.x, rd[u][dd], wx[0][dd]); wx[1][dd] = fmaf(a.y, rd[u][dd], wx[1][dd]);
                    wx[2][dd] = fmaf(a.z, rd[u][dd], wx[2][dd]); wx[3][dd] = fmaf(a.w, rd[u][dd], wx[3][dd]);
                }
            }
            *reinterpret_cast<float4*>(As + (sr + 8 * u) * P + c4) = a;
            *reinterpret_cast<float4*>(Bs + (sr + 8 * u) * P + c4) = b;
        }
    };
    if (XM == 1 || GM == 1) load_idx(r_begin);
    load_regs(r_begin);
    __syncthreads();
    write_lds(0, r_begin);
    if (r_begin + KT < r_end) load_regs(r_begin + KT);
    __syncthreads();
    int it = 0;
    for (int rb0 = r_begin; rb0 < r_end; rb0 += KT, ++it) {
        const float* As = smem + (it & 1) * STAGE + half * P + wm * 64 + l31;
        const float* Bs = smem + (it & 1) * STAGE + KT * P + half * P + wn * 64 + l31;
#pragma unroll
        for (int s = 0; s < KT / 2; ++s) {
            const float a0 = As[2 * s * P], a1 = As[2 * s * P + 32];
            const float b0 = Bs[2 * s * P], b1 = Bs[2 * s * P + 32];
            acc[0][0] = __builtin_amdgcn_mfma_f32_32x32x2f32(a0, b0, acc[0][0], 0, 0, 0);
            acc[0][1] = __builtin_amdgcn_mfma_f32_32x32x2f32(a0, b1, acc[0][1], 0, 0, 0);
            acc[1][0] = __builtin_amdgcn_mfma_f32_32x32x2f32(a1, b0, acc[1][0], 0, 0, 0);
            acc[1][1] = __builtin_amdgcn_mfma_f32_32x32x2f32(a1, b1, acc[1][1], 0, 0, 0);
        }
        if (rb0 + KT < r_end) write_lds(it + 1, rb0 + KT);
        if (rb0 + 2 * KT < r_end) load_regs(rb0 + 2 * KT);
        __syncthreads();
    }
    float* pout = partial + (size_t)blockIdx.y * n_out * Kp;
#pragma unroll
    for (int a = 0; a < 2; ++a)
#pragma unroll
        for (int b = 0; b < 2; ++b)
#pragma unroll
            for (int v = 0; v < 16; ++v) {
                const int n = n0 + wm * 64 + a * 32 + acc_row(v, half), k = k0 + wn * 64 + b * 32 + l31;
                pout[(size_t)n * Kp + k] = acc[a][b][v];
            }
    if (coords) {
        float* red = smem;
#pragma unroll
        for (int j = 0; j < 4; ++j)
#pragma unroll
            for (int dd = 0; dd < 3; ++dd) red[(sr * BT + c4 + j) * 3 + dd] = wx[j][dd];
        __syncthreads();
        for (int i = tid; i < BT * 3; i += 256) {
            float sum = 0.f;
#pragma unroll
            for (int q = 0; q < 8; ++q) sum += red[q * BT * 3 + i];
            pout[(size_t)(n0 + i / 3) * Kp + x.feat_c + i % 3] = sum;
        }
    }
}

template <int XM, int GM>
__global__ __launch_bounds__(256, 1) void gemm_dw_wide_split_kernel(DzSrc d, XSrc x, const int32_t* __restrict__ n_rows_dev,
                                                                    int n_rows_static, int Kp, int n_out, int tiles_k,
                                                                    float* __restrict__ partial, unsigned long long* __restrict__ ts) {
    KTimer kt_(ts);
    constexpr int BT = 128, OPL = BT * 64, STAGE = 6 * OPL, VM = 512;
    __shared__ __attribute__((aligned(16))) unsigned char smem_b[2 * STAGE];
    __shared__ __attribute__((aligned(16))) float vP[5 * VM];
    float* sv = vP + 3 * VM;
    float* tv = sv + VM;
    const int tid = threadIdx.x, lane = tid & 63;
    const int wave = __builtin_amdgcn_readfirstlane(tid >> 6);
    const int wm = wave >> 1, wn = wave & 1;
    const int l31 = lane & 31, half = lane >> 5;
    const int n0 = (blockIdx.x / tiles_k) * BT, k0 = (blockIdx.x % tiles_k) * BT;
    const int n_rows = n_rows_dev ? min(*n_rows_dev, n_rows_static) : n_rows_static;
    int chunk = gad_cdiv_dev(n_rows, (int)gridDim.y);
    chunk = (chunk + KT - 1) / KT * KT;
    const int r_begin = blockIdx.y * chunk, r_end = min(r_begin + chunk, n_rows);
    if (r_begin >= r_end) return;
    for (int i = tid; i < BT; i += 256) {
        float Pc, Qc, Sc;
        dz_coef(d, n0 + i, Pc, Qc, Sc, blockIdx.y == 0 && k0 == 0);
        vP[i] = Pc; vP[VM + i] = Qc; vP[2 * VM + i] = Sc;
        if (XM == 0) { sv[i] = x.scale[k0 + i]; tv[i] = x.shift[k0 + i]; }
    }
    const bool coords = XM == 1 && k0 == 0;
    float wx[4][3];
#pragma unroll
    for (int j = 0; j < 4; ++j) { wx[j][0] = 0.f; wx[j][1] = 0.f; wx[j][2] = 0.f; }
    f32x16 acc[2][2], an[2][2];
#pragma unroll
    for (int a = 0; a < 2; ++a)
#pragma unroll
        for (int b = 0; b < 2; ++b)
#pragma unroll
            for (int v = 0; v < 16; ++v) { acc[a][b][v] = 0.f; an[a][b][v] = 0.f; }
    const int rq = tid & 7, c4 = (tid >> 3) * 4;
    const float sgn = rq >= 4 ? -1.f : 1.f;
    const int gpitch = GM == 0 ? d.g_pitch : d.c;
    float4 rz[4], rg[4], rx[4];
    int4 ra[4];
    float rw[4], rd[4][3];
    int pq[4], gq[4], gd[4];
    auto load_idx = [&](int rb0) {
#pragma unroll
        for (int u = 0; u < 4; ++u) {
            const int r = rb0 + 4 * rq + u;
            const int rr = r < r_end ? r : r_end - 1;
            pq[u] = XM == 1 ? x.row_pt[rr] : 0;
            gq[u] = (XM == 1 && x.ctr_xyz) ? x.row_grp[rr] : 0;
            gd[u] = GM == 1 ? d.row_grp[rr] : 0;
        }
    };
    auto load_regs = [&](int rb0) {
#pragma unroll
        for (int u = 0; u < 4; ++u) {
            const int r = rb0 + 4 * rq + u;
            const int rr = r < r_end ? r : r_end - 1;
            rw[u] = d.row_w ? d.row_w[rr] : 1.f;
            rz[u] = ldg4(d.z + (size_t)rr * d.z_pitch + n0 + c4);
            if (GM == 0) {
                rg[u] = ldg4(d.G + (size_t)rr * gpitch + n0 + c4);
            } else {
                const int grp = gd[u];
                ra[u] = *reinterpret_cast<const int4*>(d.argmax + (size_t)grp * gpitch + n0 + c4);
                rg[u] = ldg4(d.dout + (size_t)grp * gpitch + n0 + c4);
            }
            if (XM == 0) {
                rx[u] = ldg4(x.zin + (size_t)rr * x.zin_pitch + k0 + c4);
            } else {
                rx[u] = ldg4(x.feat + (size_t)pq[u] * x.feat_c + k0 + c4);
                if (coords) {
                    const float* p = x.src_xyz + (size_t)pq[u] * 3;
                    float q0 = p[0], q1 = p[1], q2 = p[2];
                    if (x.ctr_xyz) {
                        const float* cp = x.ctr_xyz + (size_t)gq[u] * 3;
                        q0 = __fsub_rn(q0, cp[0]); q1 = __fsub_rn(q1, cp[1]); q2 = __fsub_rn(q2, cp[2]);
                    }
                    rd[u][0] = q0; rd[u][1] = q1; rd[u][2] = q2;
                }
            }
        }
        if (XM == 1 || GM == 1) load_idx(rb0 + KT);
    };
    const int wr_off = c4 * 64 + (rq & 1) * 8, wr_q = rq >> 1;
    auto write_lds = [&](int it, int rb0) {
        unsigned char* As = smem_b + (it & 1) * STAGE;
        unsigned char* Bs = As + 3 * OPL;
        const float4 Pv = *reinterpret_cast<const float4*>(vP + c4), Qv = *reinterpret_cast<const float4*>(vP + VM + c4);
        const float4 Sv = *reinterpret_cast<const float4*>(vP + 2 * VM + c4);
        float4 s4 = f4zero(), t4 = f4zero();
        if (XM == 0) { s4 = *reinterpret_cast<const float4*>(sv + c4); t4 = *reinterpret_cast<const float4*>(tv + c4); }
        float av[4][4], bv[4][4];
#pragma unroll
        for (int u = 0; u < 4; ++u) {
            const int r = rb0 + 4 * rq + u;
            float4 g = rg[u];
            const float4 z = rz[u];
            if (GM == 1) {
                g.x = ra[u].x == r ? g.x : 0.f; g.y = ra[u].y == r ? g.y : 0.f;
                g.z = ra[u].z == r ? g.z : 0.f; g.w = ra[u].w == r ? g.w : 0.f;
            }
            const float w = rw[u];
            float4 a, b;
            a.x = Pv.x * g.x - w * fmaf(Sv.x, z.x, Qv.x); a.y = Pv.y * g.y - w * fmaf(Sv.y, z.y, Qv.y);
            a.z = Pv.z * g.z - w * fmaf(Sv.z, z.z, Qv.z); a.w = Pv.w * g.w - w * fmaf(Sv.w, z.w, Qv.w);
            if (XM == 0) {
                b.x = fmaxf(fmaf(rx[u].x, s4.x, t4.x), 0.f); b.y = fmaxf(fmaf(rx[u].y, s4.y, t4.y), 0.f);
                b.z = fmaxf(fmaf(rx[u].z, s4.z, t4.z), 0.f); b.w = fmaxf(fmaf(rx[u].w, s4.w, t4.w), 0.f);
            } else {
                b = rx[u];
            }
            if (r >= r_end) { a = f4zero(); b = f4zero(); }
            if (coords) {
#pragma unroll
                for (int dd = 0; dd < 3; ++dd) {
                    wx[0][dd] = fmaf(a.x, rd[u][dd], wx[0][dd]); wx[1][dd] = fmaf(a.y, rd[u][dd], wx[1][dd]);
                    wx[2][dd] = fmaf(a.z, rd[u][dd], wx[2][dd]); wx[3][dd] = fmaf(a.w, rd[u][dd], wx[3][dd]);
                }
            }
            av[u][0] = a.x * sgn; av[u][1] = a.y * sgn; av[u][2] = a.z * sgn; av[u][3] = a.w * sgn;
            bv[u][0] = b.x; bv[u][1] = b.y; bv[u][2] = b.z; bv[u][3] = b.w;
        }
#pragma unroll
        for (int j = 0; j < 4; ++j) {
            const int off = wr_off + j * 64 + (((wr_q ^ (((c4 + j) >> 2) & 3))) << 4);
            unsigned h0, m0, l0, h1, m1, l1;
            gad_split2(av[0][j], av[1][j], h0, m0, l0);
            gad_split2(av[2][j], av[3][j], h1, m1, l1);
            *reinterpret_cast<uint2*>(As + off) = make_uint2(h0, h1);
            *reinterpret_cast<uint2*>(As + OPL + off) = make_uint2(m0, m1);
            *reinterpret_cast<uint2*>(As + 2 * OPL + off) = make_uint2(l0, l1);
            gad_split2(bv[0][j], bv[1][j], h0, m0, l0);
            gad_split2(bv[2][j], bv[3][j], h1, m1, l1);
            *reinterpret_cast<uint2*>(Bs + off) = make_uint2(h0, h1);
            *reinterpret_cast<uint2*>(Bs + OPL + off) = make_uint2(m0, m1);
            *reinterpret_cast<uint2*>(Bs + 2 * OPL + off) = make_uint2(l0, l1);
        }
    };
    if (XM == 1 || GM == 1) load_idx(r_begin);
    load_regs(r_begin);
    __syncthreads();
    write_lds(0, r_begin);
    if (r_begin + KT < r_end) load_regs(r_begin + KT);
    __syncthreads();
    const int fo = ((half ^ ((l31 >> 2) & 3)) << 4);
    const int arow = (wm * 64 + l31) * 64, brow = 3 * OPL + (wn * 64 + l31) * 64;
    int it = 0;
    for (int rb0 = r_begin; rb0 < r_end; rb0 += KT, ++it) {
        const unsigned char* st = smem_b + (it & 1) * STAGE;
#pragma unroll
        for (int s2 = 0; s2 < 2; ++s2) {
            const int off = fo ^ (s2 << 5);
            gad_u32x4 A[2][3], B[2][3];
#pragma unroll
            for (int a = 0; a < 2; ++a)
#pragma unroll
                for (int pl = 0; pl < 3; ++pl) {
                    A[a][pl] = *reinterpret_cast<const gad_u32x4*>(st + arow + a * (32 * 64) + pl * OPL + off);
                    B[a][pl] = *reinterpret_cast<const gad_u32x4*>(st + brow + a * (32 * 64) + pl * OPL + off);
                }
#define GAD_SPD(PA, PB_)                                                                                                       \
            _Pragma("unroll") for (int a = 0; a < 2; ++a) _Pragma("unroll") for (int b = 0; b < 2; ++b) {                      \
                if (s2) an[a][b] = __builtin_amdgcn_mfma_f32_32x32x16_bf16(gad_as_bf16x8(A[a][PA]), gad_as_bf16x8(B[b][PB_]), an[a][b], 0, 0, 0); \
                else acc[a][b] = __builtin_amdgcn_mfma_f32_32x32x16_bf16(gad_as_bf16x8(A[a][PA]), gad_as_bf16x8(B[b][PB_]), acc[a][b], 0, 0, 0); \
            }
            GAD_SPD(2, 0) GAD_SPD(0, 2) GAD_SPD(1, 1) GAD_SPD(1, 0) GAD_SPD(0, 1) GAD_SPD(0, 0)
#undef GAD_SPD
        }
        if (rb0 + KT < r_end) write_lds(it + 1, rb0 + KT);
        if (rb0 + 2 * KT < r_end) load_regs(rb0 + 2 * KT);
        __syncthreads();
    }
    float* pout = partial + (size_t)blockIdx.y * n_out * Kp;
#pragma unroll
    for (int a = 0; a < 2; ++a)
#pragma unroll
        for (int b = 0; b < 2; ++b)
#pragma unroll
            for (int v = 0; v < 16; ++v) {
                const int n = n0 + wm * 64 + a * 32 + acc_row(v, half), k = k0 + wn * 64 + b * 32 + l31;
                pout[(size_t)n * Kp + k] = acc[a][b][v] - an[a][b][v];
            }
    if (coords) {
        float* red = reinterpret_cast<float*>(smem_b);
#pragma unroll
        for (int j = 0; j < 4; ++j)
#pragma unroll
            for (int dd = 0; dd < 3; ++dd) red[(rq * BT + c4 + j) * 3 + dd] = wx[j][dd];
        __syncthreads();
        for (int i = tid; i < BT * 3; i += 256) {
            float sum = 0.f;
#pragma unroll
            for (int q = 0; q < 8; ++q) sum += red[q * BT * 3 + i];
            pout[(size_t)(n0 + i / 3) * Kp + x.feat_c + i % 3] = sum;
        }
    }
}

static bool dw_wideable(const gad_gemm_dw_args& a, int k_used, bool vec) {
    const gad_gemm_fwd_args& in = a.in;
    const gad_dz_src& d = a.dz;
    if (g_opt_deterministic || !g_opt_dw_wide || !vec || in.n_groups != 1 || in.zin_off[0] != 0 || a.dz_off[0] != 0) return false;
    if (in.n_rows < 2048 || in.n_out[0] % 128 != 0 || in.n_out[0] > 512 || in.ones_col >= 0) return false;
    if (in.mode == 1) {
        if (g_opt_dw_wide == 2 || d.gmode != 0 || in.act_c != 0 || in.feat_c % 128 != 0 || in.feat_c > 512) return false;
        if (in.Kp != ((in.feat_c + 3 + 7) & ~7) || k_used != in.feat_c + 3) return false;
    } else {
        if (in.Kp % 128 != 0 || in.Kp > 512 || k_used != in.Kp) return false;
        if (in.c_in != in.Kp || !in.scale || !in.shift || !in.relu || in.extra) return false;
    }
    if (!d.z || d.z_pitch % 4 != 0 || !d.relu || !d.premasked || !(d.coefP && d.coefQ && d.coefS)) return false;
    if (d.gmode == 0 ? (d.g_pitch % 4 != 0 || !d.G) : (d.c % 4 != 0)) return false;
    return a.partial != nullptr && a.row_splits <= 0;
}

static bool dw_gather_streamable(const gad_gemm_dw_args& a, int k_used) {
    const gad_gemm_fwd_args& in = a.in;
    const gad_dz_src& d = a.dz;
    if (g_opt_deterministic || !g_opt_dw_stream || in.mode != 1 || in.n_groups != 1 || in.Kp > 32 || in.n_out[0] != 64 || k_used > in.Kp) return false;
    if (in.zin_off[0] != 0 || a.dz_off[0] != 0 || in.n_rows < 32768 || d.gmode != 0 || !d.G) return false;
    if (!d.z || !d.scale || !d.relu || !d.premasked || !(d.coefP && d.coefQ && d.coefS)) return false;
    if (in.feat_c + 3 + (in.action ? in.act_c : 0) > in.Kp) return false;
    if (!a.partial || 256ll * 64 * in.Kp > a.partial_elems) return false;
    return a.row_splits <= 0;
}

static bool dw_streamable(const gad_gemm_dw_args& a, int k_used) {
    const gad_gemm_fwd_args& in = a.in;
    const gad_dz_src& d = a.dz;
    if (g_opt_deterministic || !g_opt_dw_stream || in.mode != 0 || in.n_groups != 1 || in.Kp != 64 || in.c_in != 64 || k_used != 64) return false;
    if (in.zin_off[0] != 0 || a.dz_off[0] != 0 || (in.n_out[0] != 64 && in.n_out[0] != 128)) return false;
    if (in.n_rows < 32768 || !in.scale || !in.shift || !in.relu || in.extra || in.ones_col >= 0) return false;
    if (!d.z || !d.scale || !d.relu || !d.premasked || !(d.coefP && d.coefQ && d.coefS)) return false;
    if (d.gmode != 0 && d.c != in.n_out[0]) return false;
    if (!a.partial || (long long)DW_STREAM_SPLITS * in.n_out[0] * 64 > a.partial_elems) return false;
    return a.row_splits <= 0;
}

static float* det_dw_slab(long long elems, void* stream) {
    float* p = static_cast<float*>(gad_det_scratch(stream, GAD_DET_SLOTS2, (size_t)elems * sizeof(float)));
    if (p && hipMemsetAsync(p, 0, (size_t)elems * sizeof(float), (hipStream_t)stream) != hipSuccess) {
        gad_set_error("deterministic mode: clearing the partial dW slab failed");
        return nullptr;
    }
    return p;
}

extern "C" int gad_gemm_dw(const gad_gemm_dw_args* a, void* stream) {
    unsigned long long* ts = gad_take_timing_slot(stream);
    GAD_REQUIRE(a && a->gacc, GAD_ERR_NULL, "gemm_dw: null pointer");
    const gad_gemm_fwd_args& in = a->in;
    GAD_REQUIRE(in.n_groups >= 1 && in.n_groups <= GAD_MAX_GROUPS, GAD_ERR_SHAPE, "gemm_dw: n_groups");
    GAD_REQUIRE(in.Kp % 8 == 0, GAD_ERR_SHAPE, "gemm_dw: Kp must be a multiple of 8");
    if (int e = check_input(in, "gemm_dw")) return e;
    GAD_REQUIRE(a->dz.gmode == 0 ? a->dz.G != nullptr : (a->dz.argmax && a->dz.dout && a->dz.row_grp), GAD_ERR_NULL,
                "gemm_dw: gradient source");
    if (in.n_rows <= 0) return GAD_OK;
    XSrc x = make_xsrc(in);
    DzSrc d = make_dzsrc(a->dz);
    Groups gr = make_groups(in.n_groups, a->dz_off, in.w_off, in.zin_off, in.n_out);
    const int nmax = max_nout(gr);
    int k_used = in.mode == 0 ? in.c_in + (in.extra ? 1 : 0) : in.feat_c + 3 + in.act_c;
    if (in.ones_col >= k_used) k_used = in.ones_col + 1;
    if (k_used > in.Kp) k_used = in.Kp;
    hipStream_t st = (hipStream_t)stream;
    const int rows = in.n_rows;
    const bool vec = dz_vectorizable(a->dz, a->dz_off, in.n_out, in.n_groups);
    const bool skinny_route = !g_opt_deterministic && g_opt_dw_skinny && in.mode == 0 && a->dz.gmode == 0 && !in.n_rows_dev && rows <= 1024;
    if (a->dz.bn_dbeta && (skinny_route || dw_gather_streamable(*a, k_used) || dw_streamable(*a, k_used))) {
        gad_dz_src dz2 = a->dz;
        if (int e2 = coef_fallback(dz2, stream)) return e2;
        d = make_dzsrc(dz2);
    }
    if (skinny_route) {
        if (g_opt_skinny_nw == 4)
            hipLaunchKernelGGL(gemm_dw_skinny_kernel<4>, dim3(gad_cdiv(nmax, 32), gad_cdiv(k_used, 32), gr.n), dim3(64 * 4), 0, st, d, x,
                               gr, rows, in.Kp, k_used, a->gacc, ts);
        else
            hipLaunchKernelGGL(gemm_dw_skinny_kernel<SK_NW>, dim3(gad_cdiv(nmax, 32), gad_cdiv(k_used, 32), gr.n), dim3(64 * SK_NW), 0, st, d, x,
                               gr, rows, in.Kp, k_used, a->gacc, ts);
        GAD_CHECK_LAUNCH("gemm_dw(skinny)");
        return GAD_OK;
    }
    if (dw_gather_streamable(*a, k_used)) {
        const int splits = 256;
        const int gps = in.grp_per_sample > 0 ? in.grp_per_sample : 1;
        hipLaunchKernelGGL(gemm_dw_gather_stream_kernel, dim3(splits), dim3(512), 0, st, d, x, in.n_rows_dev, rows, splits, in.Kp, k_used,
                           1.0f / (float)gps, a->partial, ts);
        GAD_CHECK_LAUNCH("gemm_dw(gather stream)");
        hipLaunchKernelGGL(dw_reduce_kernel, dim3(gad_cdiv((long long)nmax * in.Kp, 256), gad_cdiv(splits, DW_RED_CHUNK), gr.n), dim3(256), 0,
                           st, a->partial, (long long)splits * nmax * in.Kp, gr, in.n_rows_dev, rows, splits, in.Kp, k_used, a->gacc, 1);
        GAD_CHECK_LAUNCH("dw_reduce");
        return GAD_OK;
    }
    if (dw_streamable(*a, k_used)) {
        const int splits = DW_STREAM_SPLITS;
        float* part = a->partial;
        if (in.n_out[0] == 64) {
            if (a->dz.gmode == 0) hipLaunchKernelGGL((gemm_dw_stream_kernel<1, 0>), dim3(splits), dim3(512), 0, st, d, x, in.n_rows_dev, rows, splits, part, ts);
            else                  hipLaunchKernelGGL((gemm_dw_stream_kernel<1, 1>), dim3(splits), dim3(512), 0, st, d, x, in.n_rows_dev, rows, splits, part, ts);
        } else {
            if (a->dz.gmode == 0) hipLaunchKernelGGL((gemm_dw_stream_kernel<2, 0>), dim3(splits), dim3(512), 0, st, d, x, in.n_rows_dev, rows, splits, part, ts);
            else                  hipLaunchKernelGGL((gemm_dw_stream_kernel<2, 1>), dim3(splits), dim3(512), 0, st, d, x, in.n_rows_dev, rows, splits, part, ts);
        }
        GAD_CHECK_LAUNCH("gemm_dw(stream)");
        hipLaunchKernelGGL(dw_reduce_kernel, dim3(gad_cdiv((long long)nmax * in.Kp, 256), gad_cdiv(splits, DW_RED_CHUNK), gr.n), dim3(256), 0,
                           st, part, (long long)splits * nmax * in.Kp, gr, in.n_rows_dev, rows, splits, in.Kp, k_used, a->gacc, 1);
        GAD_CHECK_LAUNCH("dw_reduce");
        return GAD_OK;
    }
    if (dw_wideable(*a, k_used, vec)) {
        const int tn_ = in.n_out[0] / 128, tk_ = (in.mode == 1 ? in.feat_c : in.Kp) / 128;
        int splits = gad_cdiv(g_opt_dw_wide_wgs, tn_ * tk_);
        const int by_rows = gad_cdiv(rows, 4 * KT);
        if (splits > by_rows) splits = by_rows;
        if (splits < 1) splits = 1;
        if ((long long)splits * in.n_out[0] * in.Kp <= a->partial_elems && split_on(GAD_SPLIT_DW_WIDE)) {
#define LAUNCH_DWS(XM, GM)                                                                                                     \
            hipLaunchKernelGGL((gemm_dw_wide_split_kernel<XM, GM>), dim3(tn_ * tk_, splits), dim3(256), 0, st, d, x, in.n_rows_dev, rows, \
                               in.Kp, in.n_out[0], tk_, a->partial, ts)
            if (in.mode == 1) LAUNCH_DWS(1, 0); else if (a->dz.gmode == 0) LAUNCH_DWS(0, 0); else LAUNCH_DWS(0, 1);
#undef LAUNCH_DWS
            GAD_CHECK_LAUNCH("gemm_dw(wide split)");
            hipLaunchKernelGGL(dw_reduce_kernel, dim3(gad_cdiv((long long)nmax * in.Kp, 256), gad_cdiv(splits, DW_RED_CHUNK), gr.n), dim3(256),
                               0, st, a->partial, (long long)splits * nmax * in.Kp, gr, in.n_rows_dev, rows, splits, in.Kp, k_used, a->gacc);
            GAD_CHECK_LAUNCH("dw_reduce");
            return GAD_OK;
        }
        if ((long long)splits * in.n_out[0] * in.Kp <= a->partial_elems) {
            if (in.mode == 1)
                hipLaunchKernelGGL((gemm_dw_wide_kernel<1, 0>), dim3(tn_ * tk_, splits), dim3(256), 0, st, d, x, in.n_rows_dev, rows, in.Kp,
                                   in.n_out[0], tk_, a->partial, ts);
            else if (a->dz.gmode == 0)
                hipLaunchKernelGGL((gemm_dw_wide_kernel<0, 0>), dim3(tn_ * tk_, splits), dim3(256), 0, st, d, x, in.n_rows_dev, rows, in.Kp,
                                   in.n_out[0], tk_, a->partial, ts);
            else
                hipLaunchKernelGGL((gemm_dw_wide_kernel<0, 1>), dim3(tn_ * tk_, splits), dim3(256), 0, st, d, x, in.n_rows_dev, rows, in.Kp,
                                   in.n_out[0], tk_, a->partial, ts);
            GAD_CHECK_LAUNCH("gemm_dw(wide)");
            hipLaunchKernelGGL(dw_reduce_kernel, dim3(gad_cdiv((long long)nmax * in.Kp, 256), gad_cdiv(splits, DW_RED_CHUNK), gr.n), dim3(256),
                               0, st, a->partial, (long long)splits * nmax * in.Kp, gr, in.n_rows_dev, rows, splits, in.Kp, k_used, a->gacc);
            GAD_CHECK_LAUNCH("dw_reduce");
            return GAD_OK;
        }
    }
    long long group_stride = 0;
#define LAUNCH_DW4(WM, WN, TM, TN, XM, V, VM)                                                              \
    hipLaunchKernelGGL((gemm_dw_kernel<WM, WN, TM, TN, XM, V, VM>), dim3(tn_ * tk_, splits, gr.n), dim3(256), 0, st, d, \
                       x, gr, in.n_rows_dev, rows, in.Kp, k_used, tk_, a->gacc, part, group_stride, ts)
#define LAUNCH_DW3(WM, WN, TM, TN, XM, V)                                                                  \
    do { if (narrow) LAUNCH_DW4(WM, WN, TM, TN, XM, V, 512); else LAUNCH_DW4(WM, WN, TM, TN, XM, V, VMAX); } while (0)
#define LAUNCH_DW(WM, WN, TM, TN)                                                                          \
    do {                                                                                                   \
        constexpr int BM = WM * TM * 32, BN = WN * TN * 32;                                                \
        const int tn_ = gad_cdiv(nmax, BM), tk_ = gad_cdiv(k_used, BN);                                    \
        splits = a->row_splits;                                                                            \
        if (splits <= 0) {                                                                                 \
            splits = gad_cdiv(512, tn_ * tk_ * gr.n);                                                                         \
            const int by_rows = gad_cdiv(rows, 8 * KT);                                                    \
            if (splits > by_rows) splits = by_rows;                                                        \
            if (splits < 1) splits = 1;                                                                    \
        }                                                                                                  \
        group_stride = (long long)splits * nmax * in.Kp;                                                   \
        if (part && (splits == 1 || group_stride * gr.n > a->partial_elems)) part = nullptr; \
        if (g_opt_deterministic) {                \
            part = splits > 1 ? det_dw_slab(group_stride * gr.n, stream) : nullptr;                       \
            if (splits > 1 && !part) return GAD_ERR_LAUNCH;                                                \
        }                                                                                                  \
        if (in.mode == 0) { if (vec) LAUNCH_DW3(WM, WN, TM, TN, 0, true); else LAUNCH_DW3(WM, WN, TM, TN, 0, false); } \
        else              { if (vec) LAUNCH_DW3(WM, WN, TM, TN, 1, true); else LAUNCH_DW3(WM, WN, TM, TN, 1, false); } \
    } while (0)
    int splits = 1;
    float* part = a->partial;
    const bool narrow = nmax <= 512 && (in.mode != 0 || in.c_in <= 512);
    if (nmax <= 32) {
        LAUNCH_DW(1, 4, 1, 1);
    } else if (k_used <= 32) {
        LAUNCH_DW(4, 1, 1, 1);
    } else {
        LAUNCH_DW(2, 2, 1, 1);
    }
#undef LAUNCH_DW
#undef LAUNCH_DW3
#undef LAUNCH_DW4
    GAD_CHECK_LAUNCH("gemm_dw");
    if (part && g_opt_deterministic) {
        for (int g = 0; g < gr.n; ++g)
            if (int e = gad_ordered_reduce(part + (size_t)g * group_stride, (long long)gr.nout[g] * in.Kp, splits,
                                           (long long)gr.nout[g] * in.Kp, a->gacc + gr.woff[g], stream)) return e;
    } else if (part) {
        hipLaunchKernelGGL(dw_reduce_kernel, dim3(gad_cdiv((long long)nmax * in.Kp, 256), gad_cdiv(splits, DW_RED_CHUNK), gr.n),
                           dim3(256), 0, st, part,
                           group_stride, gr, in.n_rows_dev, rows, splits, in.Kp, k_used, a->gacc);
        GAD_CHECK_LAUNCH("dw_reduce");
    }
    return GAD_OK;
}

template <int NIT, int GM, int L1>
__global__ __launch_bounds__(256, NIT >= 8 ? 1 : 2) void gemm_bwd_wide_kernel(DzSrc d, XSrc x, const int32_t* __restrict__ n_rows_dev,
                                                               int n_rows_static, const float* __restrict__ W, int Kp, DxEpi e,
                                                               float* __restrict__ partial, unsigned long long* __restrict__ ts) {
    KTimer kt_(ts);
    constexpr int N = NIT * 64, P = 68, TILE = 64 * P;
    __shared__ __attribute__((aligned(16))) float smem[2 * TILE + 3 * N + 64 * 4];
    __shared__ int32_t ptS[64];
    float* As = smem;
    float* Ws = smem + TILE;
    float* vP = smem + 2 * TILE;
    float* relS = vP + 3 * N;
    const int tid = threadIdx.x, lane = tid & 63;
    const int wave = __builtin_amdgcn_readfirstlane(tid >> 6);
    const int wm = wave >> 1, wn = wave & 1;
    const int l31 = lane & 31, half = lane >> 5;
    const int k0 = blockIdx.y * 64;
    const int n_rows = n_rows_dev ? min(*n_rows_dev, n_rows_static) : n_rows_static;
    const int n_tiles = (n_rows + 63) >> 6;
    const int c4 = (tid & 15) * 4, sr = tid >> 4;
    for (int i = tid; i < N; i += 256) {
        float Pc, Qc, Sc;
        dz_coef(d, i, Pc, Qc, Sc, first_workgroup());
        vP[i] = Pc; vP[N + i] = Qc; vP[2 * N + i] = Sc;
    }
    const int gpitch = GM == 0 ? d.g_pitch : d.c;
    const __amdgpu_buffer_rsrc_t zr = __builtin_amdgcn_make_buffer_rsrc(const_cast<float*>(d.z), 0, gad_nbytes(n_rows, d.z_pitch * 4), 0x00020000);
    const __amdgpu_buffer_rsrc_t gr_ = __builtin_amdgcn_make_buffer_rsrc(const_cast<float*>(GM == 0 ? d.G : d.dout), 0,
                                                                         GM == 0 ? gad_nbytes(n_rows, gpitch * 4) : GAD_BUF_MAX, 0x00020000);
    const __amdgpu_buffer_rsrc_t ar = __builtin_amdgcn_make_buffer_rsrc(const_cast<int32_t*>(GM == 0 ? d.row_grp : d.argmax), 0, GAD_BUF_MAX, 0x00020000);
    const __amdgpu_buffer_rsrc_t wr = __builtin_amdgcn_make_buffer_rsrc(const_cast<float*>(W), 0, GAD_BUF_MAX, 0x00020000);
    const __amdgpu_buffer_rsrc_t xr = __builtin_amdgcn_make_buffer_rsrc(const_cast<float*>(L1 ? x.feat : x.zin), 0,
                                                                        L1 ? GAD_BUF_MAX : gad_nbytes(n_rows, x.zin_pitch * 4), 0x00020000);
    const __amdgpu_buffer_rsrc_t sr_ = __builtin_amdgcn_make_buffer_rsrc(partial, 0, GAD_BUF_MAX, 0x00020000);
    const int zp_pitch4 = L1 ? 0 : e.zprev_pitch * 4, go_pitch4 = L1 ? 0 : e.gout_pitch * 4;
    const __amdgpu_buffer_rsrc_t pr = __builtin_amdgcn_make_buffer_rsrc(const_cast<float*>(L1 ? W : e.zprev), 0, L1 ? 0 : gad_nbytes(n_rows, zp_pitch4), 0x00020000);
    const __amdgpu_buffer_rsrc_t or_ = __builtin_amdgcn_make_buffer_rsrc(L1 ? const_cast<float*>(W) : e.gout, 0, L1 ? 0 : gad_nbytes(n_rows, go_pitch4), 0x00020000);
    const int kx = k0 + wn * 32 + l31;
    float xs = 1.f, xt = 0.f, ps = 0.f, pt = 0.f, pm = 0.f, pi = 0.f;
    if (!L1) { xs = x.scale[kx]; xt = x.shift[kx]; ps = e.ps[kx]; pt = e.pt[kx]; pm = e.pm[kx]; pi = e.pi[kx]; }
    const bool coords = L1 && k0 == 0;
    float wx[NIT][3];
    if (L1) {
#pragma unroll
        for (int it = 0; it < NIT; ++it) { wx[it][0] = 0.f; wx[it][1] = 0.f; wx[it][2] = 0.f; }
    }
    f32x16 accw[NIT];
#pragma unroll
    for (int it = 0; it < NIT; ++it)
#pragma unroll
        for (int v = 0; v < 16; ++v) accw[it][v] = 0.f;
    float cb = 0.f, cg = 0.f;
    int vw[4];
#pragma unroll
    for (int u = 0; u < 4; ++u) vw[u] = ((sr + 16 * u) * Kp + k0 + c4) * 4;
    const int xpitch4 = L1 ? x.feat_c * 4 : x.zin_pitch * 4;
    const int vx = (half * (L1 ? 0 : x.zin_pitch) + kx) * 4;
    const int vzp = (4 * half * (L1 ? 0 : e.zprev_pitch) + kx) * 4, vgo = (4 * half * (L1 ? 0 : e.gout_pitch) + kx) * 4;
    int vz[4], vg[4];
    float wrow[4];
    float4 rz[4], rg[4], rb[4];
    gad_u32x4 ra[4];
    auto meta = [&](int row0) {
#pragma unroll
        for (int u = 0; u < 4; ++u) {
            const int r = row0 + sr + 16 * u;
            const bool live = r < n_rows;
            const int rr = live ? r : max(n_rows - 1, 0);
            const float w = d.row_w ? d.row_w[rr] : 1.f;
            wrow[u] = live ? w : 0.f;
            vz[u] = (r * d.z_pitch + c4) * 4;
            vg[u] = ((GM == 1 ? d.row_grp[rr] : r) * gpitch + c4) * 4;
        }
    };
    auto load_regs = [&](int it) {
// ... 309 lines not shown
```

Baseline: 392.8.

## Fold sign flips into data, reorder A rows, use buffer loads across GEMM kernels

Several GEMM kernels stop applying per-row sign XORs during bf16 splitting. The sign is instead folded into precomputed negated coefficients, negated affine/ReLU, or a permuted A-row slot mapping. Global loads in the dz/dw kernels move to buffer-resource loads with 32-bit offsets, and a new A32 template variant is selected when sizes fit. Other changes: a prefetch is moved after the split under sched barriers, BN epilogue params are staged in LDS, and DPP and lane-id details are adjusted. The aim is to cut VALU work and address arithmetic in the hot loops, at the cost of more LDS, more template variants and subtle correctness risk in the sign handling.

```diff
diff --git a/ga-ddpg_amd/csrc/gemm.hip b/ga-ddpg_amd/csrc/gemm.hip
--- a/ga-ddpg_amd/csrc/gemm.hip
+++ b/ga-ddpg_amd/csrc/gemm.hip
@@ -687,10 +687,12 @@
 #pragma unroll
         for (int p = 0; p < 3; ++p) *reinterpret_cast<gad_u32x4*>(q + p * BPL + u * (64 * 64)) = b.r[u][p];
 }
-__device__ __forceinline__ void store_a4(unsigned char* stage, int row, int tid, float4 v, unsigned sg) {
+__device__ __forceinline__ int a_row_of_slot(int slot) { return slot < 32 ? 2 * slot : 2 * ((slot - 8) & 31) + 1; }
+__device__ __forceinline__ int a_slot_of_row(int row) { return (row & 1) ? 32 + (((row >> 1) + 8) & 31) : (row >> 1); }
+__device__ __forceinline__ void store_a4(unsigned char* stage, int row, int tid, float4 v) {
     unsigned h0, m0, l0, h1, m1, l1;
-    gad_split2(__uint_as_float(__float_as_uint(v.x) ^ sg), __uint_as_float(__float_as_uint(v.y) ^ sg), h0, m0, l0);
-    gad_split2(__uint_as_float(__float_as_uint(v.z) ^ sg), __uint_as_float(__float_as_uint(v.w) ^ sg), h1, m1, l1);
+    gad_split2(v.x, v.y, h0, m0, l0);
+    gad_split2(v.z, v.w, h1, m1, l1);
     unsigned char* q = stage + row * 64 + (((((tid & 7) >> 1) ^ ((row >> 2) & 3))) << 4) + ((tid & 1) << 3);
     *reinterpret_cast<uint2*>(q) = make_uint2(h0, h1);
     *reinterpret_cast<uint2*>(q + APL) = make_uint2(m0, m1);
@@ -761,7 +763,8 @@
 #pragma unroll
     for (int u = 0; u < 2; ++u) vbs[u] = ((n0 + (tid >> 2) + 64 * u) * wsp_pitch + (tid & 3) * 8) * 2;
     unsigned char* const smem_b = reinterpret_cast<unsigned char*>(smem);
-    const int sp_fo = ((half ^ ((l31 >> 2) & 3)) << 4);
+    const int sp_slot = spw::a_slot_of_row(wm * 32 + l31);
+    const int sp_fo = ((half ^ ((sp_slot >> 2) & 3)) << 4);
     if (XM == 0) {
         if (x.bn.stat_sum) {
             const bool writer = blockIdx.x == 0 && blockIdx.y == 0;
@@ -793,7 +796,8 @@
             psgn[0] = pe.gamma[n0 + lane] < 0.f ? -1.f : 1.f;
             psgn[1] = pe.gamma[n0 + 64 + lane] < 0.f ? -1.f : 1.f;
         }
-        const int ra0 = min(row0 + ur, max(n_rows - 1, 0)), ra1 = min(row0 + ur + 32, max(n_rows - 1, 0));
+        const int ra0 = min(row0 + (SP ? spw::a_row_of_slot(ur) : ur), max(n_rows - 1, 0));
+        const int ra1 = min(row0 + (SP ? spw::a_row_of_slot(ur + 32) : ur + 32), max(n_rows - 1, 0));
         const int va0 = ((XM == 0 ? ra0 * x.zin_pitch : x.row_pt[ra0] * x.feat_c) + c4) * 4;
         const int va1 = ((XM == 0 ? ra1 * x.zin_pitch : x.row_pt[ra1] * x.feat_c) + c4) * 4;
         float4 ra2[2][2], rb2[2][SP ? 1 : 4];
@@ -820,11 +824,16 @@
 #pragma unroll
             for (int u = 0; u < 2; ++u) {
                 float4 v = ra[u];
-                if (XM == 0) {
+                if (XM == 0 && SP && u == 1) {
+                    v.x = fminf(fmaf(v.x, -s4.x, -t4.x), -0.f); v.y = fminf(fmaf(v.y, -s4.y, -t4.y), -0.f);
+                    v.z = fminf(fmaf(v.z, -s4.z, -t4.z), -0.f); v.w = fminf(fmaf(v.w, -s4.w, -t4.w), -0.f);
+                } else if (XM == 0) {
                     v.x = fmaxf(fmaf(v.x, s4.x, t4.x), 0.f); v.y = fmaxf(fmaf(v.y, s4.y, t4.y), 0.f);
                     v.z = fmaxf(fmaf(v.z, s4.z, t4.z), 0.f); v.w = fmaxf(fmaf(v.w, s4.w, t4.w), 0.f);
+                } else if (SP && u == 1) {
+                    v.x = -v.x; v.y = -v.y; v.z = -v.z; v.w = -v.w;
                 }
-                if (SP) spw::store_a4(smem_b + (kt & 1) * spw::STAGE, ur + 32 * u, tid, v, (ur & 1) ? 0x80000000u : 0u);
+                if (SP) spw::store_a4(smem_b + (kt & 1) * spw::STAGE, ur + 32 * u, tid, v);
                 else *reinterpret_cast<float4*>(As + (ur + 32 * u) * P + c4) = v;
             }
             if (SP) { spw::store_b(smem_b + (kt & 1) * spw::STAGE, rbs[SP ? S : 0], tid); return; }
@@ -858,7 +867,7 @@
         auto ktile = [&](int kt, auto nxtc) {
             if (SP) {
                 GAD_WKL(0);
-                spw::ktile(smem_b + (kt & 1) * spw::STAGE, (wm * 32 + l31) * 64, (wn * 64 + l31) * 64, sp_fo, acc, an);
+                spw::ktile(smem_b + (kt & 1) * spw::STAGE, sp_slot * 64, (wn * 64 + l31) * 64, sp_fo, acc, an);
                 GAD_WKL(1);
                 if (kt + 1 < nk) write_lds(kt + 1, nxtc);
                 if (kt + 3 < nk) load_regs(kt + 3, nxtc);
@@ -1181,8 +1190,10 @@
     tS = (long long)kt_start;
 #endif
     for (; slab < slab_end; slab += stride) {
-        load_slab(slab + stride, pt_nxt, rn);
-        pt_nxt = load_pt(slab + 2 * stride);
+        if (!SP) {
+            load_slab(slab + stride, pt_nxt, rn);
+            pt_nxt = load_pt(slab + 2 * stride);
+        }
         float4 w4[4];
 #pragma unroll
         for (int q = 0; q < 4; ++q) {
@@ -1220,16 +1231,22 @@
                     const int c = 16 * sg + 8 * half + 4 * e;
                     const float4 s4 = *reinterpret_cast<const float4*>(sv + c), t4 = *reinterpret_cast<const float4*>(tv + c);
                     const float4 zr = ra[SP ? 2 * sg + e : 0].a;
-                    const float a0 = __builtin_fmaxf(fmaf(zr.x, s4.x, t4.x), 0.f), a1 = __builtin_fmaxf(fmaf(zr.y, s4.y, t4.y), 0.f);
-                    const float a2 = __builtin_fmaxf(fmaf(zr.z, s4.z, t4.z), 0.f), a3 = __builtin_fmaxf(fmaf(zr.w, s4.w, t4.w), 0.f);
+                    const unsigned sgn = ((sg ^ l31) & 1) ? 0x80000000u : 0u;
+                    const float a0 = __uint_as_float(__float_as_uint(__builtin_fmaxf(fmaf(zr.x, s4.x, t4.x), 0.f)) ^ sgn);
+                    const float a1 = __uint_as_float(__float_as_uint(__builtin_fmaxf(fmaf(zr.y, s4.y, t4.y), 0.f)) ^ sgn);
+                    const float a2 = __uint_as_float(__float_as_uint(__builtin_fmaxf(fmaf(zr.z, s4.z, t4.z), 0.f)) ^ sgn);
+                    const float a3 = __uint_as_float(__float_as_uint(__builtin_fmaxf(fmaf(zr.w, s4.w, t4.w), 0.f)) ^ sgn);
                     gad_split2(a0, a1, ah[2 * e], am[2 * e], al[2 * e]);
                     gad_split2(a2, a3, ah[2 * e + 1], am[2 * e + 1], al[2 * e + 1]);
                 }
-                const unsigned sgn = ((sg ^ l31) & 1) ? 0x80008000u : 0u;
-                AH[sg] = gad_u32x4{ah[0] ^ sgn, ah[1] ^ sgn, ah[2] ^ sgn, ah[3] ^ sgn};
-                AM[sg] = gad_u32x4{am[0] ^ sgn, am[1] ^ sgn, am[2] ^ sgn, am[3] ^ sgn};
-                AL[sg] = gad_u32x4{al[0] ^ sgn, al[1] ^ sgn, al[2] ^ sgn, al[3] ^ sgn};
-            }
+                AH[sg] = gad_u32x4{ah[0], ah[1], ah[2], ah[3]};
+                AM[sg] = gad_u32x4{am[0], am[1], am[2], am[3]};
+                AL[sg] = gad_u32x4{al[0], al[1], al[2], al[3]};
+            }
+            __builtin_amdgcn_sched_barrier(0);
+            load_slab(slab + stride, pt_nxt, ra);
+            pt_nxt = load_pt(slab + 2 * stride);
+            __builtin_amdgcn_sched_barrier(0);
 #pragma unroll
             for (int pp = 0; pp < TN / 2; ++pp) {
                 f32x16 an[2];
@@ -1341,8 +1358,10 @@
                 csq[t] += wz * zv;
             }
         }
-#pragma unroll
-        for (int j = 0; j < NG; ++j) ra[j] = rn[j];
+        if (!SP) {
+#pragma unroll
+            for (int j = 0; j < NG; ++j) ra[j] = rn[j];
+        }
 #ifdef GAD_X_PHASES
         GAD_PH_STAMP(tC);
         ph_top += tA - tP; ph_mfma += tB - tA; ph_epi += tC - tB; tP = tC; ++ph_n;
@@ -2384,8 +2403,9 @@
     constexpr int RB = 2 * NO + 16, WPL = 64 * RB;
     constexpr int XSL = HC * 64, XPL = 4 * XSL, XBUF = 3 * XPL;
     __shared__ __attribute__((aligned(16))) unsigned char WtS[3 * WPL];
-    __shared__ __attribute__((aligned(16))) float vec[3 * NO];
+    __shared__ __attribute__((aligned(16))) float vec[9 * NO];
     __shared__ float red[2 * 8 * 64];
+    __shared__ float pv[4 * 64];
     __shared__ __attribute__((aligned(16))) unsigned char dzb[DW ? 2 * XBUF : 16];
     const int tid = threadIdx.x, lane = tid & 63;
     const int wave = __builtin_amdgcn_readfirstlane(tid >> 6);
@@ -2411,7 +2431,10 @@
         float P, Q, S;
         dz_coef(d, i, P, Q, S, first_workgroup());
         vec[i] = P; vec[NO + i] = Q; vec[2 * NO + i] = S;
-    }
+        vec[3 * NO + i] = -P; vec[4 * NO + i] = -Q; vec[5 * NO + i] = -S;
+        vec[6 * NO + i] = 0.f; vec[7 * NO + i] = 0.f; vec[8 * NO + i] = 0.f;
+    }
+    if (tid < 64) { pv[tid] = e.ps[tid]; pv[64 + tid] = e.pt[tid]; pv[128 + tid] = e.pm[tid]; pv[192 + tid] = e.pi[tid]; }
     __syncthreads();
     const int n_slabs = (n_rows + 31) >> 5;
     const int n_quads = (n_slabs + 3) >> 2;
@@ -2421,12 +2444,6 @@
     const int nprod = DW ? 4 : 8;
 
     if (!DW || wave < 4) {
-        float ps[2], pt[2], pm[2], pi[2];
-#pragma unroll
-        for (int tk = 0; tk < 2; ++tk) {
-            const int k = tk * 32 + l31;
-            ps[tk] = e.ps[k]; pt[tk] = e.pt[k]; pm[tk] = e.pm[k]; pi[tk] = e.pi[k];
-        }
         const __amdgpu_buffer_rsrc_t grsrc = __builtin_amdgcn_make_buffer_rsrc(e.gout, 0, gad_nbytes(n_rows, 64 * 4), 0x00020000);
         float sb[2] = {0.f, 0.f}, sg[2] = {0.f, 0.f};
         constexpr int NU = NO / 8, RING = 8, AHEAD = 6, RINGG = GM == 1 ? 4 : RING, AHEADG = GM == 1 ? 2 : AHEAD;
@@ -2434,15 +2451,19 @@
         float4 rz[RING], rg[RINGG];
         int4 ra[RINGG];
         auto row_of = [&](int sl) { return min(sl < n_slabs ? sl * 32 + l31 : 0, max(n_rows - 1, 0)); };
+        const __amdgpu_buffer_rsrc_t zb_ = __builtin_amdgcn_make_buffer_rsrc(const_cast<float*>(d.z), 0, GAD_BUF_MAX, 0x00020000);
+        const __amdgpu_buffer_rsrc_t gb_ = __builtin_amdgcn_make_buffer_rsrc(const_cast<float*>(GM == 0 ? d.G : d.dout), 0, GAD_BUF_MAX, 0x00020000);
+        const __amdgpu_buffer_rsrc_t ab_ = __builtin_amdgcn_make_buffer_rsrc(const_cast<int32_t*>(GM == 1 ? d.argmax : d.row_grp), 0, GAD_BUF_MAX, 0x00020000);
         auto load_z = [&](int r, int uu) {
-            const unsigned n = 16 * (uu >> 1) + 8 * half + 4 * (uu & 1);
-            rz[uu % RING] = ldg4(d.z + ((unsigned)r * NO + n));
-            if (GM == 0) rg[uu % RINGG] = ldg4(d.G + ((unsigned)r * NO + n));
+            const int vo = (int)(((unsigned)r * NO + 8 * half) * 4u), n4 = (16 * (uu >> 1) + 4 * (uu & 1)) * 4;
+            rz[uu % RING] = buf_ld4(zb_, vo + n4, 0);
+            if (GM == 0) rg[uu % RINGG] = buf_ld4(gb_, vo + n4, 0);
         };
         auto load_g = [&](int grp, int uu) {
-            const unsigned n = 16 * (uu >> 1) + 8 * half + 4 * (uu & 1);
-            ra[uu % RINGG] = *reinterpret_cast<const int4*>(d.argmax + ((unsigned)grp * NO + n));
-            rg[uu % RINGG] = ldg4(d.dout + ((unsigned)grp * NO + n));
+            const int vo = (int)(((unsigned)grp * NO + 8 * half) * 4u), n4 = (16 * (uu >> 1) + 4 * (uu & 1)) * 4;
+            const gad_u32x4 am = __builtin_amdgcn_raw_buffer_load_b128(ab_, vo + n4, 0, 0);
+            ra[uu % RINGG] = make_int4((int)am.x, (int)am.y, (int)am.z, (int)am.w);
+            rg[uu % RINGG] = buf_ld4(gb_, vo + n4, 0);
         };
         const int round_stride = DW ? 4 * gridDim.x : 8 * gridDim.x;
         int slab = DW ? blockIdx.x * 4 + wave : wave * gridDim.x + blockIdx.x;
@@ -2457,14 +2478,14 @@
             for (int i = 0; i < AHEADG; ++i) load_g(grp_cur, i);
         }
         const unsigned psel = (l31 & 1) ? 0x03020706u : 0x05040100u;
-        const unsigned rsg = (l31 & 1) ? 0x80000000u : 0u;
+        const float* const vec_row = vec + ((l31 & 1) ? 3 * NO : 0);
         const int xq = l31 >> 3, xin = ((l31 >> 1) & 3) * 4;
         const unsigned char* const wb = WtS + l31 * RB + 16 * half;
         for (; slab < slab_limit; slab += round_stride) {
             const int r_nn = row_of(slab + 2 * round_stride);
             const int grp_nn = GM == 1 ? d.row_grp[r_nn] : 0;
             const float w_nxt = d.row_w ? d.row_w[r_nxt] : 1.f;
-            const bool row_live = slab * 32 + l31 < n_rows;
+            const float* const vecl = slab * 32 + l31 < n_rows ? vec_row : vec + 6 * NO;
             f32x16 acc[2], an[2];
 #pragma unroll
             for (int t = 0; t < 2; ++t)
@@ -2505,9 +2526,9 @@
                 for (int ee = 0; ee < 2; ++ee) {
                     const int uu = 2 * s2 + ee;
                     const int n = 16 * s2 + 8 * half + 4 * ee;
-                    const float4 P = *reinterpret_cast<const float4*>(vec + n);
-                    const float4 Q = *reinterpret_cast<const float4*>(vec + NO + n);
-                    const float4 S = *reinterpret_cast<const float4*>(vec + 2 * NO + n);
+                    const float4 P = *reinterpret_cast<const float4*>(vecl + n);
+                    const float4 Q = *reinterpret_cast<const float4*>(vecl + NO + n);
+                    const float4 S = *reinterpret_cast<const float4*>(vecl + 2 * NO + n);
                     const float4 z = rz[uu % RING];
                     float4 g = rg[uu % RINGG];
                     if (GM == 1) {
@@ -2519,9 +2540,8 @@
                     float4 a4;
                     a4.x = P.x * g.x - wrow * fmaf(S.x, z.x, Q.x); a4.y = P.y * g.y - wrow * fmaf(S.y, z.y, Q.y);
                     a4.z = P.z * g.z - wrow * fmaf(S.z, z.z, Q.z); a4.w = P.w * g.w - wrow * fmaf(S.w, z.w, Q.w);
-                    if (!row_live) a4 = make_float4(0.f, 0.f, 0.f, 0.f);
-                    gad_split2(__uint_as_float(__float_as_uint(a4.x) ^ rsg), __uint_as_float(__float_as_uint(a4.y) ^ rsg), ah[2 * ee], am[2 * ee], al[2 * ee]);
-                    gad_split2(__uint_as_float(__float_as_uint(a4.z) ^ rsg), __uint_as_float(__float_as_uint(a4.w) ^ rsg), ah[2 * ee + 1], am[2 * ee + 1], al[2 * ee + 1]);
+                    gad_split2(a4.x, a4.y, ah[2 * ee], am[2 * ee], al[2 * ee]);
+                    gad_split2(a4.z, a4.w, ah[2 * ee + 1], am[2 * ee + 1], al[2 * ee + 1]);
                 }
                 const gad_u32x4 AH = {ah[0], ah[1], ah[2], ah[3]}, AM = {am[0], am[1], am[2], am[3]}, AL = {al[0], al[1], al[2], al[3]};
                 if (DW) {
@@ -2534,7 +2554,7 @@
                         const unsigned own[3] = {ah[i], am[i], al[i]};
 #pragma unroll
                         for (int pl = 0; pl < 3; ++pl) {
-                            const unsigned nbr = (unsigned)__builtin_amdgcn_update_dpp(0, (int)own[pl], 0xB1, 0xf, 0xf, false);
+                            const unsigned nbr = (unsigned)__builtin_amdgcn_mov_dpp((int)own[pl], 0xB1, 0xf, 0xf, true);
                             *reinterpret_cast<unsigned*>(q + pl * XPL) = __builtin_amdgcn_perm(nbr, own[pl], psel);
                         }
                     }
@@ -2549,6 +2569,13 @@
                 if (DW && (s2 + 1) % (NS / 2) == 0) __syncthreads();
             }
             const bool full = slab * 32 + 32 <= n_rows;
+            __asm__ volatile("" ::: "memory");
+            float ps[2], pt[2], pm[2], pi[2];
+#pragma unroll
+            for (int tk = 0; tk < 2; ++tk) {
+                const int k = tk * 32 + l31;
+                ps[tk] = pv[k]; pt[tk] = pv[64 + k]; pm[tk] = pv[128 + k]; pi[tk] = pv[192 + k];
+            }
 #pragma unroll
             for (int v = 0; v < 16; ++v) {
                 const int row = acc_row(v, half);
@@ -2570,11 +2597,12 @@
             grp_cur = grp_nxt; grp_nxt = grp_nn;
             wrow = w_nxt;
         }
+        const int lane_e = (int)__builtin_amdgcn_mbcnt_hi(~0u, __builtin_amdgcn_mbcnt_lo(~0u, 0u));
 #pragma unroll
         for (int t = 0; t < 2; ++t) {
             const float s0 = sb[t] + __shfl_xor(sb[t], 32, 64);
             const float s1 = sg[t] + __shfl_xor(sg[t], 32, 64);
-            if (lane < 32) { red[wave * 64 + t * 32 + lane] = s0; red[(8 + wave) * 64 + t * 32 + lane] = s1; }
+            if (lane_e < 32) { red[wave * 64 + t * 32 + lane_e] = s0; red[(8 + wave) * 64 + t * 32 + lane_e] = s1; }
         }
     } else {
         const int q = wave - 4;
@@ -2647,12 +2675,13 @@
             for (int v = 0; v < 16; ++v) pout[(32 * (NCT * h + tcl) + acc_row(v, half)) * 64 + 32 * b + l31] = aw[h][v] - awn[h][v];
     }
     __syncthreads();
-    if (tid < 64) {
+    if (wave == 0) {
+        const int c = (int)__builtin_amdgcn_mbcnt_hi(~0u, __builtin_amdgcn_mbcnt_lo(~0u, 0u));
         float s0 = 0.f, s1 = 0.f;
-        for (int w = 0; w < nprod; ++w) { s0 += red[w * 64 + tid]; s1 += red[(8 + w) * 64 + tid]; }
+        for (int w = 0; w < nprod; ++w) { s0 += red[w * 64 + c]; s1 += red[(8 + w) * 64 + c]; }
         const int rep = blockIdx.x % GAD_STAT_REPLICAS;
-        atomic_add_f64(e.dbeta + (size_t)rep * e.stat_stride + tid, (double)s0);
-        atomic_add_f64(e.dgamma + (size_t)rep * e.stat_stride + tid, (double)s1);
+        atomic_add_f64(e.dbeta + (size_t)rep * e.stat_stride + c, (double)s0);
+        atomic_add_f64(e.dgamma + (size_t)rep * e.stat_stride + c, (double)s1);
     }
 }
 
@@ -2694,7 +2723,8 @@
 #pragma unroll
     for (int u = 0; u < 2; ++u) vbs[u] = ((k0out + (tid >> 2) + 64 * u) * n_out + (tid & 3) * 8) * 2;
     unsigned char* const smem_b = reinterpret_cast<unsigned char*>(smem);
-    const int sp_fo = ((half ^ ((l31 >> 2) & 3)) << 4);
+    const int sp_slot = spw::a_slot_of_row(wm * 32 + l31);
+    const int sp_fo = ((half ^ ((sp_slot >> 2) & 3)) << 4);
     for (int i = tid; i < n_out; i += 256) {
         float Pc, Qc, Sc;
         dz_coef(d, i, Pc, Qc, Sc, first_workgroup());
@@ -2720,7 +2750,7 @@
         bool live[2];
 #pragma unroll
         for (int u = 0; u < 2; ++u) {
-            const int r = row0 + ur + 32 * u;
+            const int r = row0 + (SP ? spw::a_row_of_slot(ur + 32 * u) : ur + 32 * u);
             live[u] = r < n_rows;
             const int rr = live[u] ? r : max(n_rows - 1, 0);
             wrow[u] = d.row_w ? d.row_w[rr] : 1.f;
@@ -2752,7 +2782,7 @@
                 float4 g = rg[u];
                 const float4 z = rz[u];
                 if (GM == 1) {
-                    const unsigned r = row0 + ur + 32 * u;
+                    const unsigned r = row0 + (SP ? spw::a_row_of_slot(ur + 32 * u) : ur + 32 * u);
                     g.x = ra[u].x == r ? g.x : 0.f; g.y = ra[u].y == r ? g.y : 0.f;
                     g.z = ra[u].z == r ? g.z : 0.f; g.w = ra[u].w == r ? g.w : 0.f;
                 }
@@ -2761,7 +2791,8 @@
                 v.x = P4.x * g.x - w * fmaf(S4.x, z.x, Q4.x); v.y = P4.y * g.y - w * fmaf(S4.y, z.y, Q4.y);
                 v.z = P4.z * g.z - w * fmaf(S4.z, z.z, Q4.z); v.w = P4.w * g.w - w * fmaf(S4.w, z.w, Q4.w);
                 if (!live[u]) v = f4zero();
-                if (SP) spw::store_a4(smem_b + (kt & 1) * spw::STAGE, ur + 32 * u, tid, v, (ur & 1) ? 0x80000000u : 0u);
+                if (SP && u == 1) { v.x = -v.x; v.y = -v.y; v.z = -v.z; v.w = -v.w; }
+                if (SP) spw::store_a4(smem_b + (kt & 1) * spw::STAGE, ur + 32 * u, tid, v);
                 else *reinterpret_cast<float4*>(As + (ur + 32 * u) * P + c4) = v;
             }
             if (SP) { spw::store_b(smem_b + (kt & 1) * spw::STAGE, rbs, tid); return; }
@@ -2777,7 +2808,7 @@
         __syncthreads();
         for (int kt = 0; kt < nk; ++kt) {
             if (SP) {
-                spw::ktile(smem_b + (kt & 1) * spw::STAGE, (wm * 32 + l31) * 64, (wn * 64 + l31) * 64, sp_fo, acc, an);
+                spw::ktile(smem_b + (kt & 1) * spw::STAGE, sp_slot * 64, (wn * 64 + l31) * 64, sp_fo, acc, an);
                 if (kt + 1 < nk) write_lds(kt + 1);
                 if (kt + 2 < nk) load_regs(kt + 2);
                 __syncthreads();
@@ -4051,7 +4082,7 @@
     }
 }
 
-template <int XM, int GM>
+template <int XM, int GM, bool A32>
 __global__ __launch_bounds__(256, 1) void gemm_dw_wide_split_kernel(DzSrc d, XSrc x, const int32_t* __restrict__ n_rows_dev,
                                                                     int n_rows_static, int Kp, int n_out, int tiles_k,
                                                                     float* __restrict__ partial, unsigned long long* __restrict__ ts) {
@@ -4075,8 +4106,10 @@
         float Pc, Qc, Sc;
         dz_coef(d, n0 + i, Pc, Qc, Sc, blockIdx.y == 0 && k0 == 0);
         vP[i] = Pc; vP[VM + i] = Qc; vP[2 * VM + i] = Sc;
+        vP[BT + i] = -Pc; vP[VM + BT + i] = -Qc; vP[2 * VM + BT + i] = -Sc;
         if (XM == 0) { sv[i] = x.scale[k0 + i]; tv[i] = x.shift[k0 + i]; }
     }
+    static_assert(2 * BT <= VM, "the negated coefficient copies share the vectors' slots");
     const bool coords = XM == 1 && k0 == 0;
     float wx[4][3];
 #pragma unroll
@@ -4090,12 +4123,40 @@
             for (int v = 0; v < 16; ++v) { acc[a][b][v] = 0.f; an[a][b][v] = 0.f; }
     const int rq = tid & 7, c4 = (tid >> 3) * 4;
     const float sgn = rq >= 4 ? -1.f : 1.f;
+    const float* const vPl = vP + (rq >= 4 ? BT : 0) + c4;
+    const float zero_s = __uint_as_float(rq >= 4 ? 0x80000000u : 0u);
     const int gpitch = GM == 0 ? d.g_pitch : d.c;
+    const int zp4 = d.z_pitch * 4, gp4 = gpitch * 4, xp4 = (XM == 0 ? x.zin_pitch : x.feat_c) * 4;
+    const __amdgpu_buffer_rsrc_t zb_ = __builtin_amdgcn_make_buffer_rsrc(const_cast<float*>(d.z), 0, A32 ? gad_nbytes(r_end, zp4) : 0, 0x00020000);
+    const __amdgpu_buffer_rsrc_t gb_ = __builtin_amdgcn_make_buffer_rsrc(const_cast<float*>(GM == 0 ? d.G : d.dout), 0,
+                                                                         !A32 ? 0 : GM == 0 ? gad_nbytes(r_end, gp4) : GAD_BUF_MAX, 0x00020000);
+    const __amdgpu_buffer_rsrc_t ab_ = __builtin_amdgcn_make_buffer_rsrc(const_cast<int32_t*>(GM == 1 ? d.argmax : d.row_grp), 0,
+                                                                         A32 && GM == 1 ? GAD_BUF_MAX : 0, 0x00020000);
+    const __amdgpu_buffer_rsrc_t xb_ = __builtin_amdgcn_make_buffer_rsrc(const_cast<float*>(XM == 0 ? x.zin : x.feat), 0,
+                                                                         !A32 ? 0 : XM == 0 ? gad_nbytes(r_end, xp4) : GAD_BUF_MAX, 0x00020000);
+    const __amdgpu_buffer_rsrc_t wb_ = __builtin_amdgcn_make_buffer_rsrc(const_cast<float*>(d.row_w ? d.row_w : d.z), 0,
+                                                                         A32 && d.row_w ? gad_nbytes(r_end, 4) : 0, 0x00020000);
+    const __amdgpu_buffer_rsrc_t ig_ = __builtin_amdgcn_make_buffer_rsrc(const_cast<int32_t*>(d.row_grp), 0, A32 && GM == 1 ? gad_nbytes(r_end, 4) : 0, 0x00020000);
+    const __amdgpu_buffer_rsrc_t ip_ = __builtin_amdgcn_make_buffer_rsrc(const_cast<int32_t*>(x.row_pt), 0, A32 && XM == 1 ? gad_nbytes(r_end, 4) : 0, 0x00020000);
+    const __amdgpu_buffer_rsrc_t iq_ = __builtin_amdgcn_make_buffer_rsrc(const_cast<int32_t*>(x.row_grp), 0,
+                                                                         A32 && XM == 1 && x.ctr_xyz ? gad_nbytes(r_end, 4) : 0, 0x00020000);
+    const int vz0 = (4 * rq * d.z_pitch + n0 + c4) * 4, vg0 = (GM == 0 ? 4 * rq * gpitch + n0 + c4 : n0 + c4) * 4;
+    const int vx0 = (XM == 0 ? 4 * rq * x.zin_pitch + k0 + c4 : k0 + c4) * 4, vr0 = 4 * rq * 4;
     float4 rz[4], rg[4], rx[4];
     int4 ra[4];
     float rw[4], rd[4][3];
     int pq[4], gq[4], gd[4];
     auto load_idx = [&](int rb0) {
+        if (A32) {
+            const int vr = vr0 + rb0 * 4;
+#pragma unroll
+            for (int u = 0; u < 4; ++u) {
+                pq[u] = XM == 1 ? (int)__builtin_amdgcn_raw_buffer_load_b32(ip_, vr + 4 * u, 0, 0) : 0;
+                gq[u] = (XM == 1 && x.ctr_xyz) ? (int)__builtin_amdgcn_raw_buffer_load_b32(iq_, vr + 4 * u, 0, 0) : 0;
+                gd[u] = GM == 1 ? (int)__builtin_amdgcn_raw_buffer_load_b32(ig_, vr + 4 * u, 0, 0) : 0;
+            }
+            return;
+        }
 #pragma unroll
         for (int u = 0; u < 4; ++u) {
             const int r = rb0 + 4 * rq + u;
@@ -4108,11 +4169,29 @@
     auto load_regs = [&](int rb0) {
 #pragma unroll
         for (int u = 0; u < 4; ++u) {
+            if (A32) {
+                const int ro = rb0 + u;
+                rw[u] = d.row_w ? buf_ld(wb_, vr0 + ro * 4, 0) : 1.f;
+                rz[u] = buf_ld4(zb_, (int)((unsigned)vz0 + (unsigned)ro * (unsigned)zp4), 0);
+                if (GM == 0) {
+                    rg[u] = buf_ld4(gb_, (int)((unsigned)vg0 + (unsigned)ro * (unsigned)gp4), 0);
+                } else {
+                    const int vg = vg0 + (int)__umul24((unsigned)gd[u], (unsigned)gp4);
+                    const gad_u32x4 am = __builtin_amdgcn_raw_buffer_load_b128(ab_, vg, 0, 0);
+                    ra[u] = make_int4((int)am.x, (int)am.y, (int)am.z, (int)am.w);
+                    rg[u] = buf_ld4(gb_, vg, 0);
+                }
+                if (XM == 0) rx[u] = buf_ld4(xb_, (int)((unsigned)vx0 + (unsigned)ro * (unsigned)xp4), 0);
+                else rx[u] = buf_ld4(xb_, vx0 + (int)__umul24((unsigned)pq[u], (unsigned)xp4), 0);
+            }
             const int r = rb0 + 4 * rq + u;
             const int rr = r < r_end ? r : r_end - 1;
-            rw[u] = d.row_w ? d.row_w[rr] : 1.f;
-            rz[u] = ldg4(d.z + (size_t)rr * d.z_pitch + n0 + c4);
-            if (GM == 0) {
+            if (!A32) {
+                rw[u] = d.row_w ? d.row_w[rr] : 1.f;
+                rz[u] = ldg4(d.z + (size_t)rr * d.z_pitch + n0 + c4);
+            }
+            if (A32) {
+            } else if (GM == 0) {
                 rg[u] = ldg4(d.G + (size_t)rr * gpitch + n0 + c4);
             } else {
                 const int grp = gd[u];
@@ -4120,9 +4199,9 @@
                 rg[u] = ldg4(d.dout + (size_t)grp * gpitch + n0 + c4);
             }
             if (XM == 0) {
-                rx[u] = ldg4(x.zin + (size_t)rr * x.zin_pitch + k0 + c4);
+                if (!A32) rx[u] = ldg4(x.zin + (size_t)rr * x.zin_pitch + k0 + c4);
             } else {
-                rx[u] = ldg4(x.feat + (size_t)pq[u] * x.feat_c + k0 + c4);
+                if (!A32) rx[u] = ldg4(x.feat + (size_t)pq[u] * x.feat_c + k0 + c4);
                 if (coords) {
                     const float* p = x.src_xyz + (size_t)pq[u] * 3;
                     float q0 = p[0], q1 = p[1], q2 = p[2];
@@ -4140,8 +4219,8 @@
     auto write_lds = [&](int it, int rb0) {
         unsigned char* As = smem_b + (it & 1) * STAGE;
         unsigned char* Bs = As + 3 * OPL;
-        const float4 Pv = *reinterpret_cast<const float4*>(vP + c4), Qv = *reinterpret_cast<const float4*>(vP + VM + c4);
-        const float4 Sv = *reinterpret_cast<const float4*>(vP + 2 * VM + c4);
+        const float4 Pv = *reinterpret_cast<const float4*>(vPl), Qv = *reinterpret_cast<const float4*>(vPl + VM);
+        const float4 Sv = *reinterpret_cast<const float4*>(vPl + 2 * VM);
         float4 s4 = f4zero(), t4 = f4zero();
         if (XM == 0) { s4 = *reinterpret_cast<const float4*>(sv + c4); t4 = *reinterpret_cast<const float4*>(tv + c4); }
         float av[4][4], bv[4][4];
@@ -4164,7 +4243,7 @@
             } else {
                 b = rx[u];
             }
-            if (r >= r_end) { a = f4zero(); b = f4zero(); }
+            if (r >= r_end) { a = make_float4(zero_s, zero_s, zero_s, zero_s); b = f4zero(); }
             if (coords) {
 #pragma unroll
                 for (int dd = 0; dd < 3; ++dd) {
@@ -4172,7 +4251,7 @@
                     wx[2][dd] = fmaf(a.z, rd[u][dd], wx[2][dd]); wx[3][dd] = fmaf(a.w, rd[u][dd], wx[3][dd]);
                 }
             }
-            av[u][0] = a.x * sgn; av[u][1] = a.y * sgn; av[u][2] = a.z * sgn; av[u][3] = a.w * sgn;
+            av[u][0] = a.x; av[u][1] = a.y; av[u][2] = a.z; av[u][3] = a.w;
             bv[u][0] = b.x; bv[u][1] = b.y; bv[u][2] = b.z; bv[u][3] = b.w;
         }
 #pragma unroll
@@ -4240,7 +4319,7 @@
 #pragma unroll
         for (int j = 0; j < 4; ++j)
 #pragma unroll
-            for (int dd = 0; dd < 3; ++dd) red[(rq * BT + c4 + j) * 3 + dd] = wx[j][dd];
+            for (int dd = 0; dd < 3; ++dd) red[(rq * BT + c4 + j) * 3 + dd] = wx[j][dd] * sgn;
         __syncthreads();
         for (int i = tid; i < BT * 3; i += 256) {
             float sum = 0.f;
@@ -4371,8 +4450,14 @@
         if (splits < 1) splits = 1;
         if ((long long)splits * in.n_out[0] * in.Kp <= a->partial_elems && split_on(GAD_SPLIT_DW_WIDE)) {
 #define LAUNCH_DWS(XM, GM)                                                                                                     \
-            hipLaunchKernelGGL((gemm_dw_wide_split_kernel<XM, GM>), dim3(tn_ * tk_, splits), dim3(256), 0, st, d, x, in.n_rows_dev, rows, \
-                               in.Kp, in.n_out[0], tk_, a->partial, ts)
+            do {                                                                                                               \
+                if (a32) hipLaunchKernelGGL((gemm_dw_wide_split_kernel<XM, GM, true>), dim3(tn_ * tk_, splits), dim3(256), 0, st, d, x, \
+                                            in.n_rows_dev, rows, in.Kp, in.n_out[0], tk_, a->partial, ts);                     \
+                else hipLaunchKernelGGL((gemm_dw_wide_split_kernel<XM, GM, false>), dim3(tn_ * tk_, splits), dim3(256), 0, st, d, x, \
+                                        in.n_rows_dev, rows, in.Kp, in.n_out[0], tk_, a->partial, ts);                         \
+            } while (0)
+            const bool a32 = rows < (1 << 24) && fits_i32_bytes(rows, a->dz.z_pitch, a->dz.gmode == 0 ? a->dz.g_pitch : a->dz.c,
+                                                                in.mode == 1 ? in.feat_c : in.zin_pitch, 0);
             if (in.mode == 1) LAUNCH_DWS(1, 0); else if (a->dz.gmode == 0) LAUNCH_DWS(0, 0); else LAUNCH_DWS(0, 1);
 #undef LAUNCH_DWS
             GAD_CHECK_LAUNCH("gemm_dw(wide split)");
```

After: 392.2. About the same (-0.1%).
